# DanielBrosch/SDPSymmetryReduction.jl

Measured on AMD Instinct MI355X. Metric: N x N SDP reductions/sec (admissible_subspace+blockDiagonalize) at N=4096, higher is better.
Workload: dtype int8 square (int32 acc) + f64 eigen

## Files before the change

### include/sdpsr.h

```cpp
#ifndef SDPSR_H
#define SDPSR_H

#include <stddef.h>
#include <stdint.h>

#ifdef __cplusplus
extern "C" {
#endif

#define SDPSR_VERSION_MAJOR 0
#define SDPSR_VERSION_MINOR 5

typedef struct sdpsr_ctx sdpsr_ctx;
typedef struct sdpsr_problem sdpsr_problem;

typedef enum sdpsr_status {
    SDPSR_OK = 0,
    SDPSR_INVALID_DECOMPOSITION_FIELD = 1,
    SDPSR_NUMERICAL_INCONSISTENCY = 2,
    SDPSR_DIMENSION_MISMATCH = 3,
    SDPSR_LABEL_OVERFLOW = 4,
    SDPSR_BAD_ARGUMENT = 5,
    SDPSR_HIP_ERROR = 6,
    SDPSR_SOLVER_ERROR = 7,
    SDPSR_OUT_OF_MEMORY = 8,
    SDPSR_NOT_CONVERGED = 9,
    SDPSR_BAD_STATE = 10
} sdpsr_status;

typedef enum sdpsr_mem { SDPSR_MEM_HOST = 0, SDPSR_MEM_DEVICE = 1 } sdpsr_mem;

typedef enum sdpsr_square_mode {
    SDPSR_SQUARE_AUTO = 0,
    SDPSR_SQUARE_I8 = 1,
    SDPSR_SQUARE_F32 = 2,
    SDPSR_SQUARE_F64 = 3
} sdpsr_square_mode;

typedef enum sdpsr_round_mode {
    SDPSR_ROUND_NEAREST = 0,
    SDPSR_ROUND_TRUNC = 1
} sdpsr_round_mode;

enum {
    SDPSR_FLAG_SEPARATE_REFINEMENTS = 1u << 0,
    SDPSR_FLAG_FRESH_IRREDUCIBLE_ELEMENT = 1u << 1,
    SDPSR_FLAG_ALWAYS_REORTHOGONALIZE = 1u << 2,
    SDPSR_FLAG_REFINE_NO_FUSE = 1u << 3,
    SDPSR_FLAG_UNPACK_EVERY_STEP = 1u << 4,
    SDPSR_FLAG_SPMM_ONE_BY_ONE = 1u << 5,
    SDPSR_FLAG_SINGLE_COUPLING_ELEMENT = 1u << 6,
    SDPSR_FLAG_SMALL_EIGEN_ON_DEVICE = 1u << 7,
    SDPSR_FLAG_NO_GRAPH = 1u << 8,
    SDPSR_FLAG_NO_VERIFY_SHORTCUT = 1u << 9,
    SDPSR_FLAG_FULL_BASIS_IMAGE = 1u << 10,
    SDPSR_FLAG_ALWAYS_PROJECT = 1u << 11,
    SDPSR_FLAG_SYTRD_PANELS = 1u << 12,
    SDPSR_FLAG_COUPLING_ON_HOST = 1u << 13,
    SDPSR_FLAG_SYTRD_ONE_LAUNCH = 1u << 14,
    SDPSR_FLAG_WAIT_FOR_EVERY_VERDICT = 1u << 15,
    SDPSR_FLAG_WIDE_LOOP_LABELS = 1u << 16,
    SDPSR_FLAG_MODULE_SCRATCH_FILLS = 1u << 17,
    SDPSR_FLAG_SQUARE_EVERY_VERDICT = 1u << 18,
    SDPSR_FLAG_CHECKS_IN_LOOP = 1u << 19,
    SDPSR_FLAG_LABELS_BEFORE_BLOCKDIAG = 1u << 20
};

typedef struct sdpsr_opts {
    uint32_t struct_size;
    int32_t square_mode;
    int32_t channels;
    int32_t max_iters;
    int32_t confirm_rounds;
    int32_t eig_driver;
    uint32_t flags;
    int32_t round_mode;
    int32_t basis_image_kernel;
    int32_t refine_path;
    int32_t label_bits;
    int32_t insert_wgs_per_cu;
    int32_t square_kernel;
    int32_t reserved[3];
} sdpsr_opts;

enum {
    SDPSR_T_TOTAL = 0,
    SDPSR_T_PROJECT = 1,
    SDPSR_T_SQUARE = 2,
    SDPSR_T_REFINE = 3,
    SDPSR_T_EIGEN = 4,
    SDPSR_T_ISO = 5,
    SDPSR_T_IRRED = 6,
    SDPSR_T_IMAGE = 7,
    SDPSR_T_COUNT = 8
};

int sdpsr_create(int device_id, uint64_t seed, const sdpsr_opts* opts, sdpsr_ctx** out);
void sdpsr_destroy(sdpsr_ctx* ctx);
const char* sdpsr_last_error(const sdpsr_ctx* ctx);
const char* sdpsr_status_string(int status);
int sdpsr_version(void);
int sdpsr_set_stream(sdpsr_ctx* ctx, void* hip_stream);
int sdpsr_synchronize(sdpsr_ctx* ctx);
int sdpsr_wait_stream(sdpsr_ctx* ctx, void* hip_stream);
int sdpsr_hint_symmetric_basis(sdpsr_ctx* ctx, int yes);
int sdpsr_set_seed(sdpsr_ctx* ctx, uint64_t seed);
int sdpsr_dimension_trajectory(sdpsr_ctx* ctx, int64_t* dims, int32_t capacity, int32_t* count);

int sdpsr_set_label_width(sdpsr_ctx* ctx, int bits);
int sdpsr_label_width(sdpsr_ctx* ctx);
int sdpsr_labels_convert(sdpsr_ctx* ctx, int64_t len, const void* in, int in_bits, void* out, int out_bits, int mem);

int sdpsr_partition_from_f64(sdpsr_ctx* ctx, int64_t len, const double* M,
                             uint32_t* labels, int64_t* nparts, int mem);
int sdpsr_partition_from_u32(sdpsr_ctx* ctx, int64_t len, const uint32_t* in,
                             uint32_t* labels, int64_t* nparts, int mem);
int sdpsr_partition_from_u64(sdpsr_ctx* ctx, int64_t len, const uint64_t* in,
                             uint32_t* labels, int64_t* nparts, int mem);
// ... 164 lines not shown
```

### include/sdpsr_prof.h

```cpp
#ifndef SDPSR_PROF_H
#define SDPSR_PROF_H

#include "sdpsr.h"

#ifdef __cplusplus
extern "C" {
#endif

int sdpsr_profile_kernel(sdpsr_ctx* ctx, int kind, int64_t n, int64_t aux, int reps,
                         double* ms_per_launch);
int sdpsr_profile_clock(sdpsr_ctx* ctx, int kind, int64_t n, int64_t aux, int reps, double* out);
int sdpsr_profile_host_waits(sdpsr_ctx* ctx, uint64_t* out);
int sdpsr_profile_loop_counts(sdpsr_ctx* ctx, int32_t restart, uint64_t* out);
int sdpsr_profile_band_chase(sdpsr_ctx* ctx, int64_t n, int b, const double* A_host, double* d_host, double* e_host, double* out);
int sdpsr_profile_band_reduce(sdpsr_ctx* ctx, int64_t n, int b, double* A_host, double* out);
int sdpsr_profile_sytrd_graphs(sdpsr_ctx* ctx, double* out);
int sdpsr_profile_gather_packed(sdpsr_ctx* ctx, int64_t n, int T, int64_t d, uint64_t key, const uint32_t* Lp_host, const uint32_t* Lfull_host,
                                int8_t* X_plain, int8_t* X_writing, int8_t* X_full, uint32_t* L_inout, int64_t guard);
int sdpsr_profile_verify(sdpsr_ctx* ctx, int64_t n, int T, int64_t d, int mode, const uint32_t* Lp_host, const uint32_t* first_idx_host,
                         const int32_t* C_host, const double* U_host, double coef, uint64_t key, double atol, uint32_t* out);
int sdpsr_profile_basis_constant(sdpsr_ctx* ctx, int64_t n, int r, int64_t d, const uint32_t* Lp_host, const uint32_t* first_idx_host,
                                 const double* U_host, double atol, uint32_t* out);
int sdpsr_profile_verify_pair(sdpsr_ctx* ctx, int64_t n, int64_t d, const uint32_t* Lp_host, const uint32_t* first_idx_host,
                              const double* a_host, const double* b_host, uint32_t* out);
int sdpsr_profile_initial_guess(sdpsr_ctx* ctx, int32_t restart, uint64_t* out);
int sdpsr_profile_narrow_labels(sdpsr_ctx* ctx, int32_t restart, uint64_t* out);
int sdpsr_profile_gather_packed_w(sdpsr_ctx* ctx, int64_t n, int T, int64_t d, uint64_t key, int width, const uint32_t* Lp_host, int8_t* X_plain,
                                  int8_t* X_writing, uint32_t* L_inout, int64_t guard);
int sdpsr_profile_verify_w(sdpsr_ctx* ctx, int64_t n, int T, int64_t d, int r, int width, const uint32_t* Lp_host, const uint32_t* first_idx_host,
                           const int32_t* C_host, const double* U_host, const double* coef_host, uint64_t key, double atol, uint32_t* out);
int sdpsr_profile_verify_pair_w(sdpsr_ctx* ctx, int64_t n, int64_t d, int width, const uint32_t* Lp_host, const uint32_t* first_idx_host,
                                const double* a_host, const double* b_host, uint32_t* out);
int sdpsr_profile_proj_coef_lower(sdpsr_ctx* ctx, int64_t n, int64_t r, uint64_t key, int width, const uint32_t* Lp_host, const double* U_host,
                                  double* partial_out, double* coef_out);
int sdpsr_profile_refine_source(sdpsr_ctx* ctx, int kind, int what, int64_t n, int64_t ld, int T, int r, int packed, int lab_packed, uint64_t key,
                                double atol, const double* a_host, const double* b_host, const double* U_host, const double* coef_host,
                                const void* C_host, uint32_t* L_inout, uint32_t* Lnew_inout, int64_t guard, int64_t prev_classes, int sym,
                                uint64_t* sig_out, int64_t* nparts, uint32_t* first_out, int32_t* report);
int sdpsr_profile_square_checks(sdpsr_ctx* ctx, int32_t restart, uint64_t* out);
int sdpsr_profile_deferred_checks(sdpsr_ctx* ctx, int32_t restart, uint64_t* out);
int sdpsr_profile_recorded_labels(sdpsr_ctx* ctx, int32_t restart, uint64_t* out);
int sdpsr_profile_square_check(sdpsr_ctx* ctx, int64_t n, int64_t d, int G, int T, const uint64_t* keys, int width, int write_full,
                               const uint32_t* Lp_host, const uint32_t* first_idx_host, uint8_t* ws_inout, uint64_t* layout,
                               uint32_t* verdicts_out, uint32_t* L_inout, int64_t guard);


int sdpsr_profile_gram(sdpsr_ctx* ctx, int mode, int64_t k, int64_t ma, int64_t nb, int64_t lda, int64_t ldb, int64_t mp, int64_t np,
                       const double* A_host, const double* B_host, double* C_inout, double* pinned_inout, int64_t guard, int32_t* report);
int sdpsr_profile_tall_times_small(sdpsr_ctx* ctx, int64_t n, int64_t ldi, int64_t kk, int64_t lds, int64_t ncols, double alpha, double beta,
                                   int64_t ldo, const double* In_host, const double* S_host, double* out_inout, int64_t guard);
int sdpsr_profile_label_product(sdpsr_ctx* ctx, int64_t n, int64_t d, int G, int64_t w, int64_t ldw, int64_t ldy, const uint64_t* keys,
                                const uint32_t* L_host, const double* W_host, double* Y_inout, int64_t guard, int32_t* report);
int sdpsr_profile_label_product_pair(sdpsr_ctx* ctx, int64_t n, int64_t d, int64_t w, int64_t ldw, int64_t ldy, const uint64_t* keys,
                                     const uint32_t* L_host, const double* W_host, double* Y0_inout, double* Y1_inout, int64_t guard,
                                     int32_t* report);
int sdpsr_profile_class_sums2(sdpsr_ctx* ctx, int64_t n, int64_t d, uint32_t first, int plain, const uint32_t* L_host, const double* X_host,
                              double* Y_inout, int64_t guard, int32_t* report);
int sdpsr_profile_class_sums(sdpsr_ctx* ctx, int64_t n, int64_t d, int64_t ldo, const uint32_t* L_host, const double* x_host,
                             double* out_inout, int64_t guard, int32_t* report);
int sdpsr_profile_symmetrize(sdpsr_ctx* ctx, int64_t m, int64_t ld, double* B_inout, int64_t guard);
int sdpsr_profile_extract_symmetric(sdpsr_ctx* ctx, int64_t m, int64_t mp, int64_t lds, const double* src_host, double* dst_inout, int64_t guard);
int sdpsr_profile_normalize_columns(sdpsr_ctx* ctx, int64_t n, int64_t ldx, int64_t hstride, int64_t nruns, const double* X_host,
                                    double* H_inout, double* norm_inout, int64_t guard);
int sdpsr_profile_random_vector(sdpsr_ctx* ctx, int64_t n, uint64_t key, double* x_inout, int64_t guard);


int sdpsr_profile_poison_scratch(sdpsr_ctx* ctx);
int sdpsr_profile_stacked_in_place(sdpsr_ctx* ctx, int64_t n, int64_t ldi, int64_t kk, int64_t lds, int64_t ncols, int64_t w, int64_t mcols,
                                   double* M_inout, const double* S_host, int64_t guard, int32_t* report);
int sdpsr_profile_lift(sdpsr_ctx* ctx, int64_t n, int64_t ldi, int64_t kk, int64_t lds, int64_t S1, double atol, const double* In_host,
                       const double* S_host, double* Qcm_inout, double* Qrm_inout, int64_t guard);
int sdpsr_profile_seed_vector(sdpsr_ctx* ctx, int64_t n, uint64_t key, double* x_inout, double* h_inout, double* norm_inout, int64_t guard);
int sdpsr_profile_qrm_current(sdpsr_ctx* ctx, int32_t* current);


int sdpsr_profile_cx_gather_herm(sdpsr_ctx* ctx, int64_t n, const uint32_t* L_host, uint64_t key, double* Hr_inout, double* Hi_inout, int64_t guard);
int sdpsr_profile_cx_heev(sdpsr_ctx* ctx, int route, int64_t n, const double* Hr_host, const double* Hi_host, double atol, double* w_inout,
                          double* Vr_inout, double* Vi_inout, int64_t guard, int32_t* info_out);
int sdpsr_profile_cx_block_norms(sdpsr_ctx* ctx, int route, int64_t n, const double* Hr_host, const double* Hi_host, const double* Vr_host,
                                 const double* Vi_host, const int32_t* space_of, int32_t neig, double* norms_inout, int64_t guard);
int sdpsr_profile_cx_irreducible(sdpsr_ctx* ctx, int route, int64_t n, int64_t vcols, const double* Hr_host, const double* Hi_host,
                                 const double* Vr_host, const double* Vi_host, const int32_t* desc, int32_t ncols, double atol,
                                 double* Qhat_inout, int64_t guard);


int sdpsr_profile_dense_block_norms(sdpsr_ctx* ctx, int route, int64_t n, int64_t ld, const double* A_host, const double* Q_host,
                                    const int32_t* space_of, int32_t neig, double* norms_inout, double* M_inout, double* T_inout, int64_t guard);
int sdpsr_profile_dense_cluster_norms(sdpsr_ctx* ctx, int64_t n, int64_t ld, const double* A_host, const double* Q_host,
                                      const double* evals_host, double atol, const int32_t* einfo, void* pack_inout, double* T_inout, int64_t guard);
int sdpsr_profile_dense_classes(sdpsr_ctx* ctx, int32_t neig, double* norms_inout, const int32_t* dims_host, double atol, uint64_t* stat_out,
                                double* edges_out, double* thr_out, uint64_t* bits_inout, int32_t* kpart_out, int64_t guard);
int sdpsr_profile_dense_irreducible(sdpsr_ctx* ctx, int route, int64_t n, int64_t ldq, int64_t vcols, const double* Q_host, const double* Bf_host,
                                    int64_t nf, const int32_t* desc, int32_t npairs, double* Qhat_inout, int64_t ncols, int64_t guard,
                                    int32_t* report);
int sdpsr_profile_copy_cols(sdpsr_ctx* ctx, int64_t n, int64_t count, const int32_t* src_cols, const int32_t* dst_cols, const double* src_host,
                            int64_t ld_src, int64_t scols, double* dst_inout, int64_t ld_dst, int64_t dcols, int64_t guard);
int sdpsr_profile_clamptol(sdpsr_ctx* ctx, int64_t len, double* a_inout, double atol, int64_t guard);


int sdpsr_profile_sytrd(sdpsr_ctx* ctx, int64_t n, int64_t ld, double* A_inout, double* d_inout, double* e_inout, double* tau_inout,
                        int64_t guard);
int sdpsr_profile_backtransform(sdpsr_ctx* ctx, int64_t n, int64_t ld, const double* A_host, const double* tau_host, double* Z_inout,
                                int64_t guard);
int sdpsr_profile_stedc(sdpsr_ctx* ctx, int64_t n, int64_t ld, const double* d_host, const double* e_host, double* w_inout, double* Z_inout,
                        int64_t guard);

#ifdef __cplusplus
}
#endif
#endif
// ... 1 lines not shown
```

### sdpsymmetryreduction.jl_amd/_lib.py

```python
from __future__ import annotations

import ctypes as C
import os
import re

import numpy as np

_HERE = os.path.dirname(os.path.abspath(__file__))
LIB_PATH = os.path.join(_HERE, "libsdpsr_hip.so")
PROF_LIB_PATH = os.path.join(_HERE, "libsdpsr_prof.so")
HEADER_PATH = os.path.join(os.path.dirname(_HERE), "include", "sdpsr.h")
PROF_HEADER_PATH = os.path.join(os.path.dirname(_HERE), "include", "sdpsr_prof.h")

MEM_HOST, MEM_DEVICE = 0, 1
SQUARE_AUTO, SQUARE_I8, SQUARE_F32, SQUARE_F64 = 0, 1, 2, 3
T_TOTAL, T_PROJECT, T_SQUARE, T_REFINE, T_EIGEN, T_ISO, T_IRRED, T_IMAGE, T_COUNT = range(9)
ROUND_NEAREST, ROUND_TRUNC = 0, 1
SETUP_NO_CONSTRAINTS, SETUP_CHOLESKY_QR2, SETUP_MGS = 0, 1, 2
FLAG_SEPARATE_REFINEMENTS = 1 << 0
FLAG_FRESH_IRREDUCIBLE_ELEMENT = 1 << 1
FLAG_ALWAYS_REORTHOGONALIZE = 1 << 2
FLAG_REFINE_NO_FUSE = 1 << 3
FLAG_UNPACK_EVERY_STEP = 1 << 4
FLAG_SPMM_ONE_BY_ONE = 1 << 5
FLAG_SINGLE_COUPLING_ELEMENT = 1 << 6
FLAG_SMALL_EIGEN_ON_DEVICE = 1 << 7
FLAG_NO_GRAPH = 1 << 8
FLAG_NO_VERIFY_SHORTCUT = 1 << 9
FLAG_FULL_BASIS_IMAGE = 1 << 10
FLAG_ALWAYS_PROJECT = 1 << 11
FLAG_SYTRD_PANELS = 1 << 12
FLAG_COUPLING_ON_HOST = 1 << 13
FLAG_SYTRD_ONE_LAUNCH = 1 << 14
FLAG_WAIT_FOR_EVERY_VERDICT = 1 << 15
FLAG_WIDE_LOOP_LABELS = 1 << 16
FLAG_MODULE_SCRATCH_FILLS = 1 << 17
FLAG_SQUARE_EVERY_VERDICT = 1 << 18
FLAG_CHECKS_IN_LOOP = 1 << 19
FLAG_LABELS_BEFORE_BLOCKDIAG = 1 << 20
BASIS_IMAGE_KERNELS = {"auto": 0, "two_stage": 1, "outer": 2, "chunk": 3}
BI_ROUTE_COMMUTATIVE, BI_ROUTE_BLOCKS, BI_ROUTE_TWO_STAGE, BI_ROUTE_OUTER, BI_ROUTE_CHUNK = 1, 2, 3, 4, 5
BI_ROUTE_REPAIRED, BI_ROUTE_SHORTCUT_REFUSED = 0x100, 0x200
TRI_UPPER, TRI_FULL = 0, 1
REFINE_PATHS = {"auto": 0, "hash": 1, "sort": 2, "bucket": 3, "no_mid": 4, "mid_no_first": 6}

LABEL_DTYPES = {8: np.dtype(np.uint8), 16: np.dtype(np.uint16), 32: np.dtype(np.uint32)}


def label_dtype(bits):
    try:
        return LABEL_DTYPES[int(bits)]
    except KeyError:
        raise ValueError(f"label width must be 8, 16 or 32, not {bits!r}") from None


STATUS = {
    0: "OK", 1: "INVALID_DECOMPOSITION_FIELD", 2: "NUMERICAL_INCONSISTENCY", 3: "DIMENSION_MISMATCH",
    4: "LABEL_OVERFLOW", 5: "BAD_ARGUMENT", 6: "HIP_ERROR", 7: "SOLVER_ERROR", 8: "OUT_OF_MEMORY",
    9: "NOT_CONVERGED", 10: "BAD_STATE",
}


class Opts(C.Structure):
    _fields_ = [
        ("struct_size", C.c_uint32),
        ("square_mode", C.c_int32),
        ("channels", C.c_int32),
        ("max_iters", C.c_int32),
        ("confirm_rounds", C.c_int32),
        ("eig_driver", C.c_int32),
        ("flags", C.c_uint32),
        ("round_mode", C.c_int32),
        ("basis_image_kernel", C.c_int32),
        ("refine_path", C.c_int32),
        ("label_bits", C.c_int32),
        ("insert_wgs_per_cu", C.c_int32),
        ("square_kernel", C.c_int32),
        ("reserved", C.c_int32 * 3),
    ]


def declared_symbols(header_path=HEADER_PATH):
    txt = open(header_path).read()
    txt = re.sub(r"/\*.*?\*/", "", txt, flags=re.S)
    return sorted(set(re.findall(r"\b(sdpsr_[a-z0-9_]+)\s*\(", txt)))


_lib = None


def load_library():
    global _lib
# ... 106 lines not shown


_prof = None


def load_prof_library():
    global _prof
    if _prof is not None:
        return _prof
    load_library()
    if not os.path.exists(PROF_LIB_PATH):
        raise RuntimeError(f"{PROF_LIB_PATH} is missing: build it with `make -C sdpsymmetryreduction.jl_amd/csrc`")
    lib = C.CDLL(PROF_LIB_PATH)
    vp, i64 = C.c_void_p, C.c_int64
    for name in ("sdpsr_profile_kernel", "sdpsr_profile_clock"):
        fn = getattr(lib, name)
        fn.restype = C.c_int
        fn.argtypes = [vp, C.c_int, i64, i64, C.c_int, C.POINTER(C.c_double)]
    lib.sdpsr_profile_band_chase.restype = C.c_int
    lib.sdpsr_profile_band_chase.argtypes = [vp, i64, C.c_int, vp, vp, vp, C.POINTER(C.c_double)]
    lib.sdpsr_profile_band_reduce.restype = C.c_int
    lib.sdpsr_profile_band_reduce.argtypes = [vp, i64, C.c_int, vp, C.POINTER(C.c_double)]
    lib.sdpsr_profile_host_waits.restype = C.c_int
    lib.sdpsr_profile_host_waits.argtypes = [vp, C.POINTER(C.c_uint64)]
    lib.sdpsr_profile_loop_counts.restype = C.c_int
    lib.sdpsr_profile_loop_counts.argtypes = [vp, C.c_int32, C.POINTER(C.c_uint64)]
    lib.sdpsr_profile_sytrd_graphs.restype = C.c_int
    lib.sdpsr_profile_sytrd_graphs.argtypes = [vp, C.POINTER(C.c_double)]
    lib.sdpsr_profile_gather_packed.restype = C.c_int
    lib.sdpsr_profile_gather_packed.argtypes = [vp, i64, C.c_int, i64, C.c_uint64, vp, vp, vp, vp, vp, vp, i64]
    lib.sdpsr_profile_verify.restype = C.c_int
    lib.sdpsr_profile_verify.argtypes = [vp, i64, C.c_int, i64, C.c_int, vp, vp, vp, vp, C.c_double, C.c_uint64, C.c_double,
                                         C.POINTER(C.c_uint32)]
    lib.sdpsr_profile_basis_constant.restype = C.c_int
    lib.sdpsr_profile_basis_constant.argtypes = [vp, i64, C.c_int, i64, vp, vp, vp, C.c_double, C.POINTER(C.c_uint32)]
    lib.sdpsr_profile_verify_pair.restype = C.c_int
    lib.sdpsr_profile_verify_pair.argtypes = [vp, i64, i64, vp, vp, vp, vp, C.POINTER(C.c_uint32)]
    lib.sdpsr_profile_initial_guess.restype = C.c_int
    lib.sdpsr_profile_initial_guess.argtypes = [vp, C.c_int32, C.POINTER(C.c_uint64)]
    lib.sdpsr_profile_narrow_labels.restype = C.c_int
    lib.sdpsr_profile_narrow_labels.argtypes = [vp, C.c_int32, C.POINTER(C.c_uint64)]
    lib.sdpsr_profile_gather_packed_w.restype = C.c_int
    lib.sdpsr_profile_gather_packed_w.argtypes = [vp, i64, C.c_int, i64, C.c_uint64, C.c_int, vp, vp, vp, vp, i64]
    lib.sdpsr_profile_verify_w.restype = C.c_int
    lib.sdpsr_profile_verify_w.argtypes = [vp, i64, C.c_int, i64, C.c_int, C.c_int, vp, vp, vp, vp, vp, C.c_uint64, C.c_double, C.POINTER(C.c_uint32)]
    lib.sdpsr_profile_verify_pair_w.restype = C.c_int
    lib.sdpsr_profile_verify_pair_w.argtypes = [vp, i64, i64, C.c_int, vp, vp, vp, vp, C.POINTER(C.c_uint32)]
    lib.sdpsr_profile_square_checks.restype = C.c_int
    lib.sdpsr_profile_square_checks.argtypes = [vp, C.c_int32, C.POINTER(C.c_uint64)]
    lib.sdpsr_profile_deferred_checks.restype = C.c_int
    lib.sdpsr_profile_deferred_checks.argtypes = [vp, C.c_int32, C.POINTER(C.c_uint64)]
    lib.sdpsr_profile_recorded_labels.restype = C.c_int
    lib.sdpsr_profile_recorded_labels.argtypes = [vp, C.c_int32, C.POINTER(C.c_uint64)]
    lib.sdpsr_profile_square_check.restype = C.c_int
    lib.sdpsr_profile_square_check.argtypes = [vp, i64, i64, C.c_int, C.c_int, vp, C.c_int, C.c_int, vp, vp, vp, vp, vp, vp, i64]
    lib.sdpsr_profile_proj_coef_lower.restype = C.c_int
    lib.sdpsr_profile_proj_coef_lower.argtypes = [vp, i64, i64, C.c_uint64, C.c_int, vp, vp, vp, vp]
    lib.sdpsr_profile_refine_source.restype = C.c_int
    lib.sdpsr_profile_refine_source.argtypes = [vp, C.c_int, C.c_int, i64, i64, C.c_int, C.c_int, C.c_int, C.c_int, C.c_uint64, C.c_double,
                                                vp, vp, vp, vp, vp, vp, vp, i64, i64, C.c_int, vp, C.POINTER(i64), vp, C.POINTER(C.c_int32)]
    f64, rep = C.c_double, C.POINTER(C.c_int32)
    lib.sdpsr_profile_gram.restype = C.c_int
    lib.sdpsr_profile_gram.argtypes = [vp, C.c_int, i64, i64, i64, i64, i64, i64, i64, vp, vp, vp, vp, i64, rep]
    lib.sdpsr_profile_tall_times_small.restype = C.c_int
    lib.sdpsr_profile_tall_times_small.argtypes = [vp, i64, i64, i64, i64, i64, f64, f64, i64, vp, vp, vp, i64]
    lib.sdpsr_profile_label_product.restype = C.c_int
    lib.sdpsr_profile_label_product.argtypes = [vp, i64, i64, C.c_int, i64, i64, i64, vp, vp, vp, vp, i64, rep]
    lib.sdpsr_profile_label_product_pair.restype = C.c_int
    lib.sdpsr_profile_label_product_pair.argtypes = [vp, i64, i64, i64, i64, i64, vp, vp, vp, vp, vp, i64, rep]
    lib.sdpsr_profile_class_sums2.restype = C.c_int
    lib.sdpsr_profile_class_sums2.argtypes = [vp, i64, i64, C.c_uint32, C.c_int, vp, vp, vp, i64, rep]
    lib.sdpsr_profile_class_sums.restype = C.c_int
    lib.sdpsr_profile_class_sums.argtypes = [vp, i64, i64, i64, vp, vp, vp, i64, rep]
    lib.sdpsr_profile_symmetrize.restype = C.c_int
    lib.sdpsr_profile_symmetrize.argtypes = [vp, i64, i64, vp, i64]
    lib.sdpsr_profile_extract_symmetric.restype = C.c_int
    lib.sdpsr_profile_extract_symmetric.argtypes = [vp, i64, i64, i64, vp, vp, i64]
    lib.sdpsr_profile_normalize_columns.restype = C.c_int
    lib.sdpsr_profile_normalize_columns.argtypes = [vp, i64, i64, i64, i64, vp, vp, vp, i64]
    lib.sdpsr_profile_random_vector.restype = C.c_int
    lib.sdpsr_profile_random_vector.argtypes = [vp, i64, C.c_uint64, vp, i64]
    lib.sdpsr_profile_poison_scratch.restype = C.c_int
    lib.sdpsr_profile_poison_scratch.argtypes = [vp]
    lib.sdpsr_profile_stacked_in_place.restype = C.c_int
    lib.sdpsr_profile_stacked_in_place.argtypes = [vp, i64, i64, i64, i64, i64, i64, i64, vp, vp, i64, rep]
    lib.sdpsr_profile_lift.restype = C.c_int
    lib.sdpsr_profile_lift.argtypes = [vp, i64, i64, i64, i64, i64, f64, vp, vp, vp, vp, i64]
    lib.sdpsr_profile_seed_vector.restype = C.c_int
    lib.sdpsr_profile_seed_vector.argtypes = [vp, i64, C.c_uint64, vp, vp, vp, i64]
    lib.sdpsr_profile_qrm_current.restype = C.c_int
    lib.sdpsr_profile_qrm_current.argtypes = [vp, rep]
    lib.sdpsr_profile_cx_gather_herm.restype = C.c_int
    lib.sdpsr_profile_cx_gather_herm.argtypes = [vp, i64, vp, C.c_uint64, vp, vp, i64]
    lib.sdpsr_profile_cx_heev.restype = C.c_int
    lib.sdpsr_profile_cx_heev.argtypes = [vp, C.c_int, i64, vp, vp, f64, vp, vp, vp, i64, rep]
    lib.sdpsr_profile_cx_block_norms.restype = C.c_int
    lib.sdpsr_profile_cx_block_norms.argtypes = [vp, C.c_int, i64, vp, vp, vp, vp, vp, C.c_int32, vp, i64]
    lib.sdpsr_profile_cx_irreducible.restype = C.c_int
    lib.sdpsr_profile_cx_irreducible.argtypes = [vp, C.c_int, i64, i64, vp, vp, vp, vp, vp, C.c_int32, f64, vp, i64]
    lib.sdpsr_profile_dense_block_norms.restype = C.c_int
    lib.sdpsr_profile_dense_block_norms.argtypes = [vp, C.c_int, i64, i64, vp, vp, vp, C.c_int32, vp, vp, vp, i64]
    lib.sdpsr_profile_dense_cluster_norms.restype = C.c_int
    lib.sdpsr_profile_dense_cluster_norms.argtypes = [vp, i64, i64, vp, vp, vp, f64, vp, vp, vp, i64]
    lib.sdpsr_profile_dense_classes.restype = C.c_int
    lib.sdpsr_profile_dense_classes.argtypes = [vp, C.c_int32, vp, vp, f64, vp, vp, vp, vp, vp, i64]
    lib.sdpsr_profile_dense_irreducible.restype = C.c_int
# ... 14 lines not shown
```

### sdpsymmetryreduction.jl_amd/csrc/blockdiag.cpp

```cpp
#include <algorithm>
#include <cmath>
#include <cstdio>
#include <cstdlib>
#include <cstring>

#include "host_internal.h"

using namespace sdpsr;

namespace sdpsr {
static int keep_labels(sdpsr_ctx* c, int64_t n, const uint32_t* P, int mem, bool trusted_symmetric, bool in_place, bool labels_are_u32,
                       uint32_t*& L) {
    hipStream_t s = c->stream;
    const int64_t len = n * n;
    int st = SDPSR_OK;
    const bool narrow = !labels_are_u32 && c->label_width != 32;
    in_place = in_place && mem == SDPSR_MEM_DEVICE && !narrow;
    L = in_place ? const_cast<uint32_t*>(P) : (uint32_t*)ctx_buf(c, "bd_labels", len * 4);
    if (!L) return SDPSR_OUT_OF_MEMORY;
    c->bd_labels_ext = in_place ? P : nullptr;
    c->bd_sym_labels = nullptr;
    c->bd_sym_epoch = 0;
    c->bd_trusted_symmetric = (trusted_symmetric && mem == SDPSR_MEM_DEVICE && P == L) ? L : nullptr;
    if (narrow) {
        st = labels_fetch(c, L, P, (size_t)len, mem);
        if (st) return st;
    } else if (mem == SDPSR_MEM_DEVICE) {
        if (P != L) {
            const bool fresh = c->bufs.find("bd_symflag") == c->bufs.end();
            uint32_t* sf = (uint32_t*)ctx_buf(c, "bd_symflag", 64);
            if (!sf) return SDPSR_OUT_OF_MEMORY;
            if (fresh) HIP_TRY(c, hipMemsetAsync(sf, 0, 64, s));
            if (++c->epoch_counter == 0) ++c->epoch_counter;
            launch_copy_check_symmetric(s, n, P, L, sf, c->epoch_counter);
            c->bd_sym_epoch = c->epoch_counter;
            c->bd_sym_labels = L;
        }
    } else {
        HIP_TRY(c, hipMemcpyAsync(L, P, len * 4, hipMemcpyHostToDevice, s));
        c->h2d_bytes += (size_t)len * 4;
    }
    return SDPSR_OK;
}

static int check_block_sizes(sdpsr_ctx* c, const std::vector<int32_t>& sizes, int64_t d) {
    int64_t final_dim = 0;
    for (int32_t sz : sizes) final_dim += (int64_t)sz * (sz + 1) / 2;
    if (final_dim == d) return SDPSR_OK;
    std::string szs;
    for (int32_t sz : sizes) szs += std::to_string(sz) + " ";
    return ctx_fail(c, SDPSR_DIMENSION_MISMATCH,
                    "final_dim=" + std::to_string(final_dim) + " block_sizes=[" + szs + "] expected dim(P)=" +
                        std::to_string(d) + " (rounding error: try another epsilon or try again; or the algebra is not block-diagonalizable over the reals)");
}

int block_diagonalize_impl(sdpsr_ctx* c, int64_t n, const uint32_t* P, int64_t d, double epsilon, int32_t* nblocks, int64_t* sum_sq,
                           int64_t* sum_s, double* phase_ms, int mem, bool trusted_symmetric, bool final_sync, bool in_place, bool labels_are_u32) {
    CHECK_CTX(c);
    if (!P || n < 1 || d < 0 || !(epsilon > 0)) return ctx_fail(c, SDPSR_BAD_ARGUMENT, "bad arguments");
    const int64_t len = n * n;
    int st = check_len(c, len);
    if (st) return st;
    hipStream_t s = c->stream;
    c->bd_valid = false;
    c->bd_q_valid = false;
    c->bd_qrm_current = false;
    PhaseTimer tm(c, phase_ms != nullptr);
    TotalEvents ev_total(phase_ms != nullptr, s);
    uint32_t* L = nullptr;
    st = keep_labels(c, n, P, mem, trusted_symmetric, in_place, labels_are_u32, L);
    if (st) return st;
    dbg_mark(c, "block_diagonalize: entered, labels copied");
    const double atol = epsilon;
    EigInfo info;
    std::vector<int32_t> sizes;
    int64_t S1 = 0, S = 0;
    st = DRIVER_FALLBACK;
    if (compression_eligible(c, n, d)) st = compressed_diagonalize(c, n, L, d, atol, info, sizes, S1, S, tm);
    if (st == DRIVER_FALLBACK && c->opts.eig_driver == 6)
        return ctx_fail(c, SDPSR_SOLVER_ERROR, "requested driver not applicable to this partition (" + c->err + ")");
    if (st != SDPSR_OK && st != DRIVER_FALLBACK) return st;
    if (st == DRIVER_FALLBACK) {
        flush_deferred_tail(c);
        st = dense_diagonalize(c, n, L, nullptr, atol, info, sizes, S1, S, tm, d);
        if (st) return st;
    }

    dbg_mark(c, "block_diagonalize: diagonalize done");
    c->bd_n = n;
    c->bd_d = d;
    c->bd_sizes = sizes;
    c->bd_sum_s = S1;
    c->bd_sum_sq = S;
    c->bd_q_valid = true;
    if (nblocks) *nblocks = (int32_t)sizes.size();
    if (sum_sq) *sum_sq = S;
    if (sum_s) *sum_s = S1;
    if (phase_ms) {
        const float ms = ev_total.stop(s);
        tm.collect();
        for (int i = 0; i < SDPSR_T_COUNT; ++i) phase_ms[i] = tm.acc[i];
        phase_ms[SDPSR_T_TOTAL] = ms;
    } else if (final_sync) {
        HIP_TRY(c, ctx_sync_stream(c, s));
    }
    st = check_block_sizes(c, sizes, d);
    if (st) return st;
    c->bd_valid = true;
    return SDPSR_OK;
}

struct BasisImage {
    enum Shortcut { FALL_THROUGH, DONE, DONE_SYNCED };
    enum Route { TWO_STAGE, OUTER, CHUNK };
    sdpsr_ctx* c;
    hipStream_t s;
    int64_t n, d, S1, S, len;
    uint32_t first;
    const uint32_t* L;
    const double* Qrm;
    double* out;
    double atol;
    const std::vector<int32_t>& sizes;
// ... 298 lines not shown
```

### sdpsymmetryreduction.jl_amd/csrc/compress.cpp

```cpp
#include <algorithm>
#include <cmath>
#include <cstdio>
#include <cstring>
#include <functional>

#include "host_internal.h"
#include "module_select.h"

using namespace sdpsr;

namespace {

struct Rider { double *dBs, *gps; bool have_t; };

struct Module {
    sdpsr_ctx* c;
    int64_t n, ld, d;
    const uint32_t* L;
    int wmax;
    int64_t wcap, ycap, wtot;
    double *W = nullptr, *T = nullptr, *zy = nullptr, *dout = nullptr, *Cc = nullptr, *dSm = nullptr, *Q1 = nullptr;
    int w = 1;
    std::vector<double> hG;
    int64_t saved_ld = 0;
// ... 137 lines not shown
            return ctx_fail(c, SDPSR_INVALID_DECOMPOSITION_FIELD,
                            "partition is not symmetric: decomposition over Float64 requested but the generic element has a complex spectrum");
    }
    sel = select_directions(hG.data(), ap, w, mc, tol, take_ref);
    return SDPSR_OK;
}

int Module::apply_stacked(int mc, const Selection& sel) {
    int e2 = h2d_sync(c, dSm, sel.coef.data(), (size_t)(w + mc) * sel.rank * 8);
    if (e2) return e2;
    double* V = W + (size_t)w * ld;
    const bool in_place = !parent_form() && launch_tall_times_small_rows(c->stream, n, ld, W, w + mc, dSm, w + mc, sel.rank, 1.0, 0.0, V, ld);
    if (!in_place) {
        live = mc;
        e2 = restore_fills();
        if (e2) return e2;
        launch_tall_times_small(c->stream, n, ld, W, w + mc, dSm, w + mc, sel.rank, 1.0, 0.0, Q1, ld);
        HIP_TRY(c, hipMemcpyAsync(V, Q1, (size_t)ld * sel.rank * 8, hipMemcpyDeviceToDevice, c->stream));
    }
    live = sel.rank;
    return SDPSR_OK;
}

int Module::absorb(int m, const Rider* rider, int& got) {
    got = 0;
    Selection s1, s2;
    int st = ortho_step(m, 1e-10, true, rider, s1);
    if (st) return st;
    if (dbg_on() && s1.rank > 0) fprintf(stderr, "[sdpsr] absorb(%d): rank %d, pivots %.3e .. %.3e (ratio %.1e)\n", m, s1.rank, s1.piv_max, s1.piv_min, s1.piv_max / s1.piv_min);
    first_product_intact = (s1.rank == 0);
    if (s1.rank == 0) return SDPSR_OK;
    if (w + s1.rank >= wmax) return driver_fallback(c, "module dimension exceeds " + std::to_string(wmax));
    st = apply_stacked(m, s1);
    if (st) return st;
    const double worst = std::max(s1.piv_max, s1.ref) / s1.piv_min;
    got = s1.rank;
    if (!(worst <= 1e3) || (c->opts.flags & SDPSR_FLAG_ALWAYS_REORTHOGONALIZE)) {
        st = ortho_step(s1.rank, 1e-6, false, nullptr, s2);
        got = s2.rank;
        if (st || got == 0) return st;
        st = apply_stacked(s1.rank, s2);
        if (st) return st;
    }
    w += got;
    live = 0;
    return SDPSR_OK;
}

int Module::class_sum_round() {
    if (!(class_sums_supports(n, d, ld) && basis_image_two_stage_fits(n, d, 1) && d <= ycap && d + 1 < wmax)) {
        flush_deferred_tail(c);
        return SDPSR_OK;
    }
    launch_class_sums(c->stream, n, d, L, W, W + (size_t)w * ld, ld);
    window = 0;
    int got;
    live = (int)d;
    return absorb((int)d, nullptr, got);
}

int Module::growth_round(int& got) {
    const bool fused = fused_product(w);
    int G = (fused && w <= 16) ? 4 : 2;
    while (G > 2 && (int64_t)G * w > ycap) --G;
    if ((int64_t)G * w > ycap || w >= d) G = 1;
    const int m = G * w;
    double* Y = W + (size_t)w * ld;
    live = 0;
    window = 1;
    deferred_window_close(c);
    if (lean && !(fused && small_on_host())) {
        const int e0 = restore_fills();
        if (e0) return e0;
    }
    if (!lean) HIP_TRY(c, hipMemsetAsync(Y, 0, (size_t)ld * round_up(m, 128) * 8, c->stream));
    bool batched = false;
    if (fused && G > 1 && G != 3 && G * w <= 64 && !(c->opts.flags & SDPSR_FLAG_SPMM_ONE_BY_ONE)) {
        double* part = (double*)ctx_buf(c, "cm_part", label_spmm_pair_partial_doubles(n) * 8);
        if (!part) return SDPSR_OUT_OF_MEMORY;
        uint64_t keys[4];
        const uint64_t save = c->stream_counter;
        for (int gidx = 0; gidx < G; ++gidx) keys[gidx] = next_key(c);
        batched = launch_label_spmm_multi(c->stream, n, L, keys, G, d, W, ld, w, part, Y, ld);
        if (!batched) c->stream_counter = save;
    }
    spec_b2 = false;
    Rider rider{};
    bool armed = false;
    if (G == 1 && small_on_host()) {
        char* pinb = (char*)ctx_pinned(c, spec_b2_offset() + (size_t)w * w * 8);
        rider.dBs = (double*)ctx_buf(c, "cm_bsmall", (size_t)64 * 64 * 8);
        rider.gps = (double*)ctx_buf(c, "gram_partials", gram_small_partial_doubles(n, 128, 128) * 8);
        armed = pinb && rider.dBs && rider.gps;
    }
    if (armed && fused && !(c->opts.flags & SDPSR_FLAG_SPMM_ONE_BY_ONE)) {
        double* part = (double*)ctx_buf(c, "cm_part", label_spmm_pair_partial_doubles(n) * 8);
        if (!part) return SDPSR_OUT_OF_MEMORY;
        uint64_t keys[2];
        const uint64_t save = c->stream_counter;
        keys[0] = next_key(c);
        keys[1] = next_key(c);
        rider.have_t = launch_label_spmm_pair(c->stream, n, L, keys, d, W, ld, w, part, Y, ld, T, ld);
        if (!rider.have_t) c->stream_counter = save;
    }
    for (int gidx = 0; gidx < G && !batched && !rider.have_t; ++gidx) {
        live = gidx * w;
        int e2 = apply_generic(w, Y + (size_t)gidx * w * ld);
// ... 198 lines not shown
```

### sdpsymmetryreduction.jl_amd/csrc/ctx.cpp

```cpp
#include <algorithm>
#include <cmath>
#include <complex>
#include <cstdio>
#include <cstdlib>
#include <cstring>
#include <chrono>
#include <functional>
#include <numeric>

#include "host_internal.h"

using namespace sdpsr;
int ctx_fail(sdpsr_ctx* c, int status, const std::string& msg) {
    if (c) c->err = std::string(sdpsr_status_string(status)) + ": " + msg;
    return status;
}

void* ctx_buf(sdpsr_ctx* c, const char* name, size_t bytes) {
    if (bytes == 0) bytes = 16;
    auto it = c->bufs.find(std::string_view(name));
    if (it != c->bufs.end() && it->second.bytes >= bytes) return it->second.p;
    DevBuf& b = it != c->bufs.end() ? it->second : c->bufs[std::string(name)];
    const std::string_view nm(name);
    if (nm == "adm_lpacked" || nm == "adm_lpacked8" || nm == "ref_first" || nm == "adm_lfull_rec") c->initial_record = InitialRecord{};
    if (nm == "adm_symflag") c->symflag_zero = false;
    if (nm == "bd_qhat" || nm == "bd_qrm") c->bd_qrm_current = false;
    if (b.p) {
        flush_deferred_tail(c);
        ctx_sync_stream(c, c->stream);
        hipFree(b.p);
        b.p = nullptr;
        b.bytes = 0;
    }
    size_t want = bytes + (bytes >> 3);
    want = (want + 255) & ~size_t(255);
    if (hipMalloc(&b.p, want) != hipSuccess) {
        b.p = nullptr;
        if (hipMalloc(&b.p, bytes) != hipSuccess) {
            b.p = nullptr;
            ctx_fail(c, SDPSR_OUT_OF_MEMORY, std::string("hipMalloc ") + name + " " + std::to_string(bytes));
            return nullptr;
        }
        want = bytes;
    }
    b.bytes = want;
    return b.p;
}


namespace sdpsr {
uint64_t steady_ns() {
    return (uint64_t)std::chrono::duration_cast<std::chrono::nanoseconds>(std::chrono::steady_clock::now().time_since_epoch()).count();
}
void* ctx_pinned(sdpsr_ctx* c, size_t bytes) {
    if (c->pinned_bytes >= bytes) return c->pinned;
    ctx_sync_stream(c, c->stream);
    if (c->pinned) hipHostFree(c->pinned);
    c->pinned = nullptr;
    c->pinned_bytes = 0;
    size_t want = std::max<size_t>(bytes + bytes / 4, 1 << 16);
    if (hipHostMalloc(&c->pinned, want, hipHostMallocCoherent) != hipSuccess) {
        c->pinned = nullptr;
        return nullptr;
    }
    c->pinned_bytes = want;
    return c->pinned;
}

bool ctx_ensure_side(sdpsr_ctx* c) {
    if (!c->side_stream && hipStreamCreateWithFlags(&c->side_stream, hipStreamNonBlocking) != hipSuccess) {
        c->side_stream = nullptr;
        (void)hipGetLastError();
        return false;
    }
    hipEvent_t* evs[] = {&c->ev_fork, &c->ev_join, &c->ev_bt_fork, &c->ev_bt_join};
    for (hipEvent_t* e : evs)
        if (!*e && hipEventCreateWithFlags(e, hipEventDisableTiming) != hipSuccess) {
// ... 257 lines not shown
```

### sdpsymmetryreduction.jl_amd/csrc/host_internal.h

```cpp
#pragma once
#include <algorithm>
#include <cstring>
#include <functional>
#include <string>
#include <vector>

#include "agree_plan.h"
#include "csr_canon.h"
#include "iso_classes.h"
#include "sdpsr_internal.h"

struct sdpsr_comm {
    int device = 0;
    int32_t world = 1, rank = 0;
    void* nccl = nullptr;
};

namespace sdpsr {

bool dbg_on();
void dbg_mark(sdpsr_ctx* c, const char* what);

struct DeviceGuard {
    int prev = -1;
// ... 189 lines not shown
constexpr PinnedWords PINNED_VERIFY{128, 1};
constexpr PinnedWords PINNED_SPECULATIVE{144, 1};
constexpr PinnedWords PINNED_BASIS_CONSTANT{192, 1};
constexpr PinnedWords PINNED_SAMPLE{224, 4};
constexpr size_t PINNED_FIXED_BYTES = 1024;
constexpr PinnedWords PINNED_BASIS_IMAGE_VERDICTS{64, 1};
constexpr PinnedWords PINNED_SMALL_FLAG{0, 1};
constexpr PinnedWords PINNED_SMALL_LABEL_CHECK{2, 2};
constexpr PinnedWords PINNED_SMALL_ROWSPACE_NNZ{4, 2};
constexpr PinnedWords PINNED_SMALL_DEFERRED_VERIFY{8, 1};
constexpr PinnedWords PINNED_SMALL_DEFERRED_SPECULATIVE{24, 1};
constexpr PinnedWords PINNED_SMALL_DEFERRED_INITIAL{16, 1};
constexpr PinnedWords PINNED_SMALL_DEFERRED_NARROW{20, 1};
constexpr PinnedWords PINNED_SMALL_GRAM_STAMP{32, 1};
constexpr PinnedWords PINNED_SMALL_CANON{44, 18};
constexpr PinnedWords PINNED_SMALL_NARROW{40, 1};
constexpr bool pinned_words_disjoint(std::initializer_list<PinnedWords> w, size_t bytes) {
    for (const PinnedWords* a = w.begin(); a != w.end(); ++a) {
        if (a->count == 0 || (a->first + a->count) * 4 > bytes) return false;
        for (const PinnedWords* b = w.begin(); b != a; ++b)
            if (a->first < b->first + b->count && b->first < a->first + a->count) return false;
    }
    return true;
}
static_assert(pinned_words_disjoint({PINNED_REFINE, PINNED_SYMMETRY, PINNED_BASIS_IMAGE_VERDICTS, PINNED_VERIFY, PINNED_SPECULATIVE, PINNED_BASIS_CONSTANT, PINNED_SAMPLE}, PINNED_FIXED_BYTES) &&
              PINNED_FIXED_BYTES % sizeof(double) == 0, "two reports share a word of c->pinned, or one reaches into the symmetry probe's doubles");
static_assert(pinned_words_disjoint({PINNED_SMALL_FLAG, PINNED_SMALL_LABEL_CHECK, PINNED_SMALL_ROWSPACE_NNZ, PINNED_SMALL_DEFERRED_VERIFY, PINNED_SMALL_DEFERRED_SPECULATIVE, PINNED_SMALL_DEFERRED_INITIAL, PINNED_SMALL_DEFERRED_NARROW, PINNED_SMALL_GRAM_STAMP, PINNED_SMALL_NARROW, PINNED_SMALL_CANON}, 256) &&
              (PINNED_SMALL_CANON.first * 4) % 8 == 0 && PINNED_SMALL_CANON.count * 4 == sizeof(CanonVerdict), "two reports share a word of c->pinned_small");
inline uint32_t* pinned_report(sdpsr_ctx* c, PinnedWords w) {
    uint32_t* p = (uint32_t*)ctx_pinned(c, PINNED_FIXED_BYTES);
    return p ? p + w.first : nullptr;
}
inline uint32_t initial_guess_violated(const sdpsr_ctx* c) {
    const volatile uint32_t* ps = c->pinned_small;
    return ps[PINNED_SMALL_DEFERRED_INITIAL.first] | ps[PINNED_SMALL_DEFERRED_NARROW.first];
}

int refine_signatures(sdpsr_ctx* c, int64_t len, const SigSource& src_in, uint32_t* labels, int64_t* nparts, int64_t sym_n = 0,
                      uint32_t* symflag_dev = nullptr, int* sym_out = nullptr, bool early = false);
int refine_signatures(sdpsr_ctx* c, int64_t len, const uint64_t* sig, uint32_t* labels, int64_t* nparts, int64_t sym_n = 0,
                      uint32_t* symflag_dev = nullptr, int* sym_out = nullptr, bool early = false);

int admissible_subspace_impl(sdpsr_ctx* c, int64_t n, const double* CL, const double* X0L, const double* U, int64_t r, double atol,
                             uint32_t* P_out, int64_t* dim_out, int32_t* iters_out, double* phase_ms, int mem, int mem_out,
                             bool final_sync, int* labels_sym_out);
int setup_mgs(sdpsr_ctx* c, int64_t len, int64_t m, double* R, double* U, double* partial, int nblk, double* coef,
              std::vector<std::vector<double>>& coeffs, std::vector<int64_t>& piv, int64_t* r_out);
std::vector<double> min_norm_coefficients(int64_t r, const std::vector<int64_t>& piv, const std::vector<std::vector<double>>& coeffs,
                                          const double* b);
int setup_tail(sdpsr_ctx* c, int64_t n, int64_t r, const double* U, const std::vector<double>& y, double atol, double* v1, double* v2,
               double* dCL, double* dX0, double* partial, int nblk, double* coef);
int block_diagonalize_impl(sdpsr_ctx* c, int64_t n, const uint32_t* P, int64_t d, double epsilon, int32_t* nblocks, int64_t* sum_sq,
                           int64_t* sum_s, double* phase_ms, int mem, bool trusted_symmetric, bool final_sync, bool in_place = false,
                           bool labels_are_u32 = true);

struct EigInfo {
    std::vector<double> vals;
    std::vector<int> ptrs;
    std::vector<int> kpart;
    bool t_valid = false;
};

struct ElemGen {
    std::function<int(double* dst)> make;
    std::function<int(double* dst)> prefetch;
    std::function<int()> join;
    std::function<int()> fork;
};
int make_element(sdpsr_ctx* c, const ElemGen* gen, int64_t n, int64_t ld, const uint32_t* L, double* dst);
int isomorphism_classes(sdpsr_ctx* c, const std::vector<double>& norms, int neig, double atol, std::vector<int>& kpart);
struct CouplingTrace {
    double edges[17];
    double thr;
};
int isomorphism_classes_device(sdpsr_ctx* c, unsigned long long* dnorms, int neig, const std::vector<int32_t>& dims, double atol,
                               std::vector<int>& kpart, CouplingTrace* trace = nullptr);
void couple_block_norms(hipStream_t s, int64_t n, int64_t ld, double* Ap, const double* Q, double* Tp, const int32_t* dspace, int neig,
                        unsigned long long* dnorms);
bool irreducible_pairs_fit_lds(int64_t max_m2);
int irreducible_pairs(sdpsr_ctx* c, int64_t n, int64_t ld, const double* Q, const double* Bf, const std::vector<int32_t>& pairs,
                      int64_t max_m2, double* Qhat, int route = -1, int* ran = nullptr);
int irreducible_pairs_one_by_one(sdpsr_ctx* c, int64_t n, int64_t ld, const double* Q, const double* Bf, const std::vector<int32_t>& pairs,
                                 double* Qhat);
int eigen_decomposition_device(sdpsr_ctx* c, int64_t n, const uint32_t* L, double atol, EigInfo& info, PhaseTimer& tm,
                               const ElemGen* gen = nullptr, int64_t expect_dim = -1);
constexpr int DRIVER_FALLBACK = -1000;
int driver_fallback(sdpsr_ctx* c, const std::string& why);
int dense_diagonalize(sdpsr_ctx* c, int64_t n, const uint32_t* L, const ElemGen* gen, double atol, EigInfo& info,
                      std::vector<int32_t>& sizes, int64_t& S1, int64_t& S, PhaseTimer& tm, int64_t expect_dim = -1);
int gemm_tn_splitk(sdpsr_ctx* c, int64_t m, int64_t n, int64_t k, const double* A, int64_t lda, const double* B, int64_t ldb,
                   double* C, int64_t ldc, const char* partials = "splitk_partials");
bool gram_tn_is_skinny(int64_t ma, int64_t nb);
int gram_tn(sdpsr_ctx* c, int64_t ma, int64_t nb, int64_t k, const double* A, int64_t lda, const double* B, int64_t ldb, double* C,
            int64_t mp, int64_t np, double* host_C = nullptr, bool* host_filled = nullptr);
int compressed_diagonalize(sdpsr_ctx* c, int64_t n, const uint32_t* L, int64_t d, double atol, EigInfo& info,
                           std::vector<int32_t>& sizes, int64_t& S1, int64_t& S, PhaseTimer& tm);
bool compression_eligible(const sdpsr_ctx* c, int64_t n, int64_t d);

int host_syev(int n, const double* A, int lda, double* w, double* Z, int ldz);
void host_count_edges17(const double* x, size_t n, const double* ed, int64_t* hist);
void host_gemm_tn(int m, int n, int k, const double* A, int lda, const double* B, int ldb, double* C, int ldc);
int murota_small_host(sdpsr_ctx* c, int w, const double* B1, const std::function<int(double*)>& next_element, double atol,
                      int64_t expect_dim, std::vector<int32_t>& sizes, int64_t& S1, int64_t& S, std::vector<double>& Qs);

void launch_symmetrize(hipStream_t s, int64_t m, int64_t ld, double* B);
void launch_extract_symmetric(hipStream_t s, int64_t m, int64_t mp, const double* src, int64_t lds_, double* dst);
void launch_splitk_reduce(hipStream_t s, int64_t len, int Z, int64_t stride, const double* P, double* C);
// ... 109 lines not shown
```

### sdpsymmetryreduction.jl_amd/csrc/kernels_blockdiag.hip

```cpp
#include <cstdlib>
#include <type_traits>
#include "host_internal.h"
#include "kernel_util.h"

namespace sdpsr {

typedef double v4d __attribute__((ext_vector_type(4)));

__global__ void block_norms_kernel(int64_t n, int64_t ld, const double* __restrict__ M,
                                   const int32_t* __restrict__ space_of, int neig,
                                   unsigned long long* __restrict__ norms) {
    const int64_t len = n * n;
    const int64_t stride = (int64_t)gridDim.x * blockDim.x;
    for (int64_t e0 = (int64_t)blockIdx.x * blockDim.x; e0 < len; e0 += stride) {
        const int64_t e = e0 + threadIdx.x;
        bool valid = e < len;
        int64_t j = valid ? e / n : 0, i = valid ? e - j * n : 0;
        int bi = space_of[i], bj = space_of[j];
        unsigned long long v = valid ? (unsigned long long)__double_as_longlong(fabs(M[i + j * ld])) : 0ull;
        int key = bi * neig + bj;
        int prev_key = __shfl_up(key, 1, 64);
        bool head = ((threadIdx.x & 63) == 0) || prev_key != key;
#pragma unroll
        for (int o = 1; o < 64; o <<= 1) {
// ... 688 lines not shown
                    for (int g2 = 1; g2 < groups; ++g2) tot += __shfl(t, jl + g2 * sub, 64);
                    t = tot;
                }
                if (act && g == 0) {
                    if (lower && diag == (uint32_t)i) t = fma(0.5, Qrm[(int64_t)r * S1 + (int64_t)j * VEC + v], t);
                    T[((int64_t)(i - 1) * nn + r) * S1 + (int64_t)j * VEC + v] = t;
                }
            }
        }
    }
}

__global__ void __launch_bounds__(256)
basis_image_blocks_kernel(int n, int S1, int64_t S, const double* __restrict__ Qrm, const double* __restrict__ T,
                          const int32_t* __restrict__ colA, const int32_t* __restrict__ colB, double atol,
                          double* __restrict__ out) {
    __shared__ double red[256];
    const int i = blockIdx.x;
    const int64_t o = (int64_t)blockIdx.y * 4 + (threadIdx.x & 3);
    const int g = threadIdx.x >> 2;
    const double* Ti = T + (int64_t)i * n * S1;
    double a0 = 0, a1 = 0;
    if (o < S) {
        const int ca = colA[o], cb = colB[o];
        int r = g;
        for (; r + 64 < n; r += 128) {
            const double qa0 = Qrm[(int64_t)r * S1 + ca], qb0 = Qrm[(int64_t)r * S1 + cb];
            const double ta0 = Ti[(int64_t)r * S1 + ca], tb0 = Ti[(int64_t)r * S1 + cb];
            const double qa1 = Qrm[(int64_t)(r + 64) * S1 + ca], qb1 = Qrm[(int64_t)(r + 64) * S1 + cb];
            const double ta1 = Ti[(int64_t)(r + 64) * S1 + ca], tb1 = Ti[(int64_t)(r + 64) * S1 + cb];
            a0 = fma(qa0, tb0, a0);
            a0 = fma(qb0, ta0, a0);
            a1 = fma(qa1, tb1, a1);
            a1 = fma(qb1, ta1, a1);
        }
        for (; r < n; r += 64) {
            a0 = fma(Qrm[(int64_t)r * S1 + ca], Ti[(int64_t)r * S1 + cb], a0);
            a0 = fma(Qrm[(int64_t)r * S1 + cb], Ti[(int64_t)r * S1 + ca], a0);
        }
    }
    red[threadIdx.x] = a0 + a1;
    __syncthreads();
    if (threadIdx.x < 4 && o < S) {
        double v = 0;
        for (int gg = 0; gg < 64; ++gg) v += red[gg * 4 + threadIdx.x];
        out[(int64_t)i * S + o] = (fabs(v) < atol) ? 0.0 : v;
    }
}

bool basis_image_two_stage_fits(int64_t n, int64_t d, int64_t S1) {
    return n <= 65535 && (2 * (d + 2) * 4 + n * 2) <= 60 * 1024 && d * n * S1 * 8 <= ((int64_t)4 << 30);
}

__global__ void __launch_bounds__(256)
class_sums_small_d_kernel(int n, int d, uint32_t first, int tstride, const uint32_t* __restrict__ L, const double* __restrict__ x,
                          double* __restrict__ out, int64_t ldo) {
    extern __shared__ __attribute__((aligned(16))) double cs_smem[];
    double* sx = cs_smem;
    const int lane = threadIdx.x & 63, wave = threadIdx.x >> 6;
    double* acc = cs_smem + n + (size_t)wave * 64 * tstride;
    double* mine = acc + (size_t)lane * tstride;
    for (int c = threadIdx.x; c < n; c += 256) sx[c] = x[c];
    __syncthreads();
    const int rows_per_round = gridDim.x * 4;
    const int bpr = (n + 511) / 512;
    const int my_rows = (n - blockIdx.x * 4 + rows_per_round - 1) / rows_per_round;
    const int total = my_rows * bpr;
    auto fetch = [&](int bq, uint32_t (&lab)[8]) {
        const int rr = bq / bpr, bb = bq - rr * bpr;
        const int r = blockIdx.x * 4 + rr * rows_per_round + wave;
        const uint32_t* col = L + (int64_t)((bq < total && r < n) ? r : 0) * n;
#pragma unroll
        for (int u = 0; u < 8; ++u) {
            const int c = bb * 512 + u * 64 + lane;
            lab[u] = col[c < n ? c : n - 1];
        }
    };
    auto process = [&](int bq, const uint32_t (&lab)[8]) {
        if (bq >= total) return;
        const int rr = bq / bpr, bb = bq - rr * bpr;
        if (bb == 0)
            for (int i = 0; i <= d; ++i) mine[i] = 0.0;
        double vv[8];
#pragma unroll
        for (int u = 0; u < 8; ++u) {
            const int c = bb * 512 + u * 64 + lane;
            vv[u] = c < n ? sx[c] : 0.0;
        }
#pragma unroll
        for (int u = 0; u < 8; ++u) atomicAdd(&mine[window_label(lab[u], first, (uint32_t)d)], vv[u]);
        if (bb == bpr - 1) {
            const int r = blockIdx.x * 4 + rr * rows_per_round + wave;
            __syncthreads();
            if (r < n)
                for (int i = 1 + lane; i <= d; i += 64) {
                    double t = 0;
                    for (int l2 = 0; l2 < 64; ++l2) t += acc[(size_t)l2 * tstride + i];
                    out[(int64_t)(i - 1) * ldo + r] = t;
                }
            __syncthreads();
        }
    };
    uint32_t qa[8], qb[8], qc[8], qd[8];
    fetch(0, qa);
    fetch(1, qb);
    fetch(2, qc);
#pragma unroll 1
    for (int bq = 0; bq < total; bq += 4) {
        fetch(bq + 3, qd);
        process(bq, qa);
        fetch(bq + 4, qa);
        process(bq + 1, qb);
        fetch(bq + 5, qb);
        process(bq + 2, qc);
        fetch(bq + 6, qc);
        process(bq + 3, qd);
    }
}

__device__ __forceinline__ double bi_weight(uint64_t key, int k) {
    return 0.5 + (double)(sdpsr_fmix64(key + 0x9E3779B97F4A7C15ULL * (uint64_t)(k + 1)) >> 11) * (1.0 / 9007199254740992.0);
}

__global__ void bi_signed_sums_kernel(int n, int S1, const double* __restrict__ Qrm, uint64_t key, double2* __restrict__ X, uint32_t* flag) {
    const int r = blockIdx.x * blockDim.x + threadIdx.x;
    if (blockIdx.x == 0)
        for (int k = threadIdx.x; k <= S1; k += blockDim.x) flag[k] = 0u;
    if (r >= n) return;
    double a = 0, b = 0;
    for (int k = 0; k < S1; ++k) {
        const double q = Qrm[(int64_t)r * S1 + k];
        a += q;
        b = fma(bi_weight(key, k), q, b);
    }
    X[r] = make_double2(a, b);
}

__global__ void bi_pair_vector_kernel(int n, int S1, const double* __restrict__ Qrm, int k1, int k2, double2* __restrict__ X) {
    const int r = blockIdx.x * blockDim.x + threadIdx.x;
    if (r < n) X[r] = make_double2(Qrm[(int64_t)r * S1 + k1], Qrm[(int64_t)r * S1 + k2]);
}

__global__ void __launch_bounds__(256)
bi_contract_pair_kernel(int n, int S1, const double* __restrict__ Qrm, const double2* __restrict__ Y, int k1, int k2, double atol,
                        double* __restrict__ out) {
    __shared__ double red[2][256];
    const int i = blockIdx.x;
    const double2* Yi = Y + (int64_t)i * n;
    double a0 = 0, a1 = 0;
    for (int r = threadIdx.x; r < n; r += 256) {
        const double2 y = Yi[r];
        a0 = fma(Qrm[(int64_t)r * S1 + k1], y.x, a0);
        a1 = fma(Qrm[(int64_t)r * S1 + k2], y.y, a1);
    }
    red[0][threadIdx.x] = a0;
    red[1][threadIdx.x] = a1;
    __syncthreads();
    if (threadIdx.x < 2) {
        double v = 0;
        for (int g = 0; g < 256; ++g) v += red[threadIdx.x][g];
        const int k = threadIdx.x == 0 ? k1 : k2;
        out[(int64_t)i * S1 + k] = (fabs(v) < atol) ? 0.0 : v;
    }
}

template <int W, bool WIN>
__global__ void __launch_bounds__(64 * W)
class_sums2_kernel(int n, int d, uint32_t first, int tstride, const uint32_t* __restrict__ L, const double2* __restrict__ X,
                   double2* __restrict__ out) {
    extern __shared__ __attribute__((aligned(16))) double2 cs2_smem[];
    const int lane = threadIdx.x & 63, wave = threadIdx.x >> 6;
    double2* acc = cs2_smem + (size_t)wave * 64 * tstride;
    double2* mine = acc + (size_t)lane * tstride;
    const int rows_per_round = gridDim.x * W;
    const int bpr = (n + 511) / 512;
    const int my_rows = (n - (int)blockIdx.x * W + rows_per_round - 1) / rows_per_round;
    const int total = my_rows * bpr;
    auto fetch = [&](int bq, uint32_t (&lab)[8], double2 (&xv)[8]) {
        const int rr = bq / bpr, bb = bq - rr * bpr;
        const int r = blockIdx.x * W + rr * rows_per_round + wave;
        const uint32_t* col = L + (int64_t)((bq < total && r < n) ? r : 0) * n;
#pragma unroll
        for (int u = 0; u < 8; ++u) {
            const int c = bb * 512 + u * 64 + lane;
            const int cc = c < n ? c : n - 1;
            lab[u] = col[cc];
            xv[u] = X[cc];
        }
    };
    auto process = [&](int bq, const uint32_t (&lab)[8], const double2 (&xv)[8]) {
        if (bq >= total) return;
        const int rr = bq / bpr, bb = bq - rr * bpr;
        if (bb == 0)
            for (int i = 0; i <= d; ++i) mine[i] = make_double2(0.0, 0.0);
#pragma unroll
        for (int u = 0; u < 8; ++u) {
            const int c = bb * 512 + u * 64 + lane;
            if (c < n) {
                const uint32_t l = WIN ? window_label(lab[u], first, (uint32_t)d) : lab[u];
                double2 t = mine[l];
                t.x += xv[u].x;
                t.y += xv[u].y;
                mine[l] = t;
            }
        }
        if (bb == bpr - 1) {
            const int r = blockIdx.x * W + rr * rows_per_round + wave;
            __syncthreads();
            if (r < n)
                for (int i = 1 + lane; i <= d; i += 64) {
                    double tx = 0, ty = 0;
                    for (int l2 = 0; l2 < 64; ++l2) {
                        const double2 v = acc[(size_t)l2 * tstride + i];
                        tx += v.x;
                        ty += v.y;
                    }
                    out[(int64_t)(i - 1) * n + r] = make_double2(tx, ty);
                }
            __syncthreads();
        }
    };
    uint32_t la[8], lb[8], lc[8];
    double2 xa[8], xb[8], xc[8];
    fetch(0, la, xa);
    fetch(1, lb, xb);
#pragma unroll 1
    for (int bq = 0; bq < total; bq += 3) {
        fetch(bq + 2, lc, xc);
        process(bq, la, xa);
        fetch(bq + 3, la, xa);
        process(bq + 1, lb, xb);
        fetch(bq + 4, lb, xb);
        process(bq + 2, lc, xc);
    }
}

__global__ void __launch_bounds__(256)
bi_contract_check_kernel(int n, int S1, const double* __restrict__ Qrm, const double2* __restrict__ Y, uint64_t key, double atol,
                         double tol, double* __restrict__ out, uint32_t* __restrict__ flag) {
    __shared__ double red[2][256];
    const int i = blockIdx.x;
    const int k = blockIdx.y * 4 + (threadIdx.x & 3);
    const int g = threadIdx.x >> 2;
    const double2* Yi = Y + (int64_t)i * n;
    double a0 = 0, a1 = 0;
    if (k < S1)
        for (int r0 = g; r0 < n; r0 += 64 * 8) {
            double q[8];
            double2 y[8];
#pragma unroll
            for (int x = 0; x < 8; ++x) {
                const int r = r0 + 64 * x;
                const int rc = r < n ? r : g;
                q[x] = r < n ? Qrm[(int64_t)rc * S1 + k] : 0.0;
                y[x] = Yi[rc];
            }
#pragma unroll
            for (int x = 0; x < 8; ++x) {
                a0 = fma(q[x], y[x].x, a0);
                a1 = fma(q[x], y[x].y, a1);
            }
        }
    red[0][threadIdx.x] = a0;
    red[1][threadIdx.x] = a1;
    __syncthreads();
    if (threadIdx.x < 4 && k < S1) {
        double v0 = 0, v1 = 0;
        for (int gg = 0; gg < 64; ++gg) {
            v0 += red[0][gg * 4 + threadIdx.x];
            v1 += red[1][gg * 4 + threadIdx.x];
        }
        if (!(fabs(v0 - v1 / bi_weight(key, k)) <= tol)) {
            if (atomicExch(&flag[1 + k], 1u) == 0u) atomicAdd(&flag[0], 1u);
        }
        out[(int64_t)i * S1 + k] = (fabs(v0) < atol) ? 0.0 : v0;
    }
}

static void launch_class_sums2(hipStream_t s, int W, int g, size_t lds, int64_t n, int64_t d, uint32_t first, bool plain, int tstride, const uint32_t* L,
                               const double2* X, double2* Y) {
    if (plain && first == 1u) {
        if (W == 4) class_sums2_kernel<4, false><<<g, 256, lds, s>>>((int)n, (int)d, first, tstride, L, X, Y);
        else if (W == 2) class_sums2_kernel<2, false><<<g, 128, lds, s>>>((int)n, (int)d, first, tstride, L, X, Y);
        else class_sums2_kernel<1, false><<<g, 64, lds, s>>>((int)n, (int)d, first, tstride, L, X, Y);
    } else {
        if (W == 4) class_sums2_kernel<4, true><<<g, 256, lds, s>>>((int)n, (int)d, first, tstride, L, X, Y);
        else if (W == 2) class_sums2_kernel<2, true><<<g, 128, lds, s>>>((int)n, (int)d, first, tstride, L, X, Y);
// ... 173 lines not shown
        }
        Bs[a2][b2] = v;
    }
    __syncthreads();
    if (only < 0 && threadIdx.x < 12) {
        const int a2 = threadIdx.x % 3, t = sz + threadIdx.x / 3;
        if (a2 < sz && t < BIB_T) {
            double v = 0;
            for (int b2 = 0; b2 < sz; ++b2) v += Bs[a2][b2] * bib_weight(key, k, b2, t, sz);
            if (!(fabs(v - ys[a2][t]) <= tol)) s_bad = 1;
        }
    }
    __syncthreads();
    if (threadIdx.x == 0 && s_bad && atomicExch(&flag[1 + k], 1u) == 0u) atomicAdd(&flag[0], 1u);
    if (threadIdx.x < 9) {
        const int a2 = threadIdx.x / 3, b2 = threadIdx.x % 3;
        if (a2 < sz && b2 < sz) {
            const double v = 0.5 * (Bs[a2][b2] + Bs[b2][a2]);
            out[(int64_t)i * S + blk_off[k] + a2 + b2 * sz] = (fabs(v) < atol) ? 0.0 : v;
        }
    }
}
size_t basis_image_blocks_workspace_doubles(int64_t n, int64_t d) { return (size_t)4 * n * (d + 1) + 9 * 65536; }
bool launch_basis_image_blocks(hipStream_t s, int64_t n, int64_t d, uint32_t first, int64_t S1, int64_t S, int nblocks, const int32_t* blk_col, const int32_t* blk_size,
                               const int64_t* blk_off, const uint32_t* L, const double* Qrm, uint64_t key, int only, double atol, double tol, double* ws,
                               double* out, uint32_t* flag, bool plain) {
    const int tstride = (int)((d + 1) | 1);
    const size_t per_wave = (size_t)64 * tstride * sizeof(double2);
    int W = 4;
    while (W > 1 && per_wave * W > 150 * 1024) W >>= 1;
    if (per_wave * W > 150 * 1024 || n < 1 || n > 0x7FFFFFFF / 2 || nblocks < 1 || nblocks > 65535) return false;
    double2* X0 = reinterpret_cast<double2*>(ws);
    double2* X1 = X0 + n;
    double2* Y0 = X1 + n;
    double2* Y1 = Y0 + (size_t)d * n;
    double* ginv = reinterpret_cast<double*>(Y1 + (size_t)d * n);
    if ((size_t)S1 * BIB_T * 8 > 48 * 1024) return false;
    bib_vectors_kernel<<<(unsigned)((n + 255) / 256), 256, (size_t)S1 * BIB_T * 8, s>>>((int)n, (int)S1, nblocks, blk_col, blk_size, key, only, Qrm, X0, X1, only < 0 ? flag : nullptr, ginv);
    int g = (int)((n + W - 1) / W);
    if (g > 256) g = 256;
    const size_t lds = per_wave * W;
    for (int pass = 0; pass < 2; ++pass) {
        const double2* X = pass ? X1 : X0;
        double2* Y = pass ? Y1 : Y0;
        launch_class_sums2(s, W, g, lds, n, d, first, plain, tstride, L, X, Y);
    }
    dim3 gc((unsigned)d, only >= 0 ? 1u : (unsigned)nblocks);
    bib_contract_kernel<<<gc, 256, 0, s>>>((int)n, (int)S1, S, blk_col, blk_size, blk_off, Qrm, Y0, Y1, ginv, key, only, atol, tol, out, flag);
    return true;
}

bool blockdiag_set_device_attributes() {
    bool ok = true;
    ok &= hipSuccess == hipFuncSetAttribute(reinterpret_cast<const void*>(&class_sums2_kernel<4, false>), hipFuncAttributeMaxDynamicSharedMemorySize, 150 * 1024);
    ok &= hipSuccess == hipFuncSetAttribute(reinterpret_cast<const void*>(&class_sums2_kernel<4, true>), hipFuncAttributeMaxDynamicSharedMemorySize, 150 * 1024);
    ok &= hipSuccess == hipFuncSetAttribute(reinterpret_cast<const void*>(&class_sums2_kernel<2, false>), hipFuncAttributeMaxDynamicSharedMemorySize, 150 * 1024);
    ok &= hipSuccess == hipFuncSetAttribute(reinterpret_cast<const void*>(&class_sums2_kernel<2, true>), hipFuncAttributeMaxDynamicSharedMemorySize, 150 * 1024);
    ok &= hipSuccess == hipFuncSetAttribute(reinterpret_cast<const void*>(&class_sums2_kernel<1, false>), hipFuncAttributeMaxDynamicSharedMemorySize, 150 * 1024);
    ok &= hipSuccess == hipFuncSetAttribute(reinterpret_cast<const void*>(&class_sums2_kernel<1, true>), hipFuncAttributeMaxDynamicSharedMemorySize, 150 * 1024);
    ok &= hipSuccess == hipFuncSetAttribute(reinterpret_cast<const void*>(&class_sums_small_d_kernel),
                        hipFuncAttributeMaxDynamicSharedMemorySize, 150 * 1024);
    ok &= hipSuccess == hipFuncSetAttribute(reinterpret_cast<const void*>(&small_qtaq_block_norms_kernel),
                        hipFuncAttributeMaxDynamicSharedMemorySize, 104 * 1024);
    ok &= hipSuccess == hipFuncSetAttribute(reinterpret_cast<const void*>(&small_cluster_qtaq_block_norms_kernel),
                        hipFuncAttributeMaxDynamicSharedMemorySize, 104 * 1024);
    ok &= hipSuccess == hipFuncSetAttribute(reinterpret_cast<const void*>(&basis_image_outer_mfma_kernel),
                        hipFuncAttributeMaxDynamicSharedMemorySize, 72 * 1024);
    ok &= hipSuccess == hipFuncSetAttribute(reinterpret_cast<const void*>(&basis_image_rows_kernel<1>),
                        hipFuncAttributeMaxDynamicSharedMemorySize, 64 * 1024);
    ok &= hipSuccess == hipFuncSetAttribute(reinterpret_cast<const void*>(&basis_image_rows_kernel<2>),
                        hipFuncAttributeMaxDynamicSharedMemorySize, 64 * 1024);
    return ok;
}

bool class_sums_supports(int64_t n, int64_t d, int64_t ldo) {
    const int tstride = (int)((d + 1) | 1);
    return ldo == n || ((size_t)n + (size_t)4 * 64 * tstride) * sizeof(double) <= 150 * 1024;
}
void launch_class_sums(hipStream_t s, int64_t n, int64_t d, const uint32_t* L, const double* x, double* out, int64_t ldo, uint32_t first) {
    const int tstride = (int)((d + 1) | 1);
    const size_t lds_small = ((size_t)n + (size_t)4 * 64 * tstride) * sizeof(double);
    if (lds_small <= 150 * 1024) {
        int g = (int)((n + 3) / 4);
        if (g > 256) g = 256;
        class_sums_small_d_kernel<<<g, 256, lds_small, s>>>((int)n, (int)d, first, tstride, L, x, out, ldo);
        return;
    }
    const size_t lds = (size_t)2 * (d + 2) * 4 + (size_t)n * 2 + 16;
    basis_image_rows_kernel<1><<<(unsigned)n, 64, lds, s>>>((int)n, (int)d, first, 1, L, x, out, 0);
}

void launch_basis_image_two_stage(hipStream_t s, int64_t n, int64_t d, uint32_t first, int64_t S1, int64_t S,
                                  const uint32_t* L, const double* Qrm, double* T, const int32_t* colA,
                                  const int32_t* colB, double atol, double* out) {
    const size_t lds = (size_t)2 * (d + 2) * 4 + (size_t)n * 2 + 16;
    if (S1 % 2 == 0)
        basis_image_rows_kernel<2><<<(unsigned)n, 64, lds, s>>>((int)n, (int)d, first, (int)S1, L, Qrm, T, 1);
    else
        basis_image_rows_kernel<1><<<(unsigned)n, 64, lds, s>>>((int)n, (int)d, first, (int)S1, L, Qrm, T, 1);
    dim3 g((unsigned)d, (unsigned)((S + 3) / 4));
    basis_image_blocks_kernel<<<g, 256, 0, s>>>((int)n, (int)S1, S, Qrm, T, colA, colB, atol, out);
}

__global__ void transpose_to_rowmajor_kernel(int64_t n, int64_t S1, const double* __restrict__ Qcm,
                                             double* __restrict__ Qrm) {
    const int64_t total = n * S1;
    const int64_t stride = (int64_t)gridDim.x * blockDim.x;
    for (int64_t t = (int64_t)blockIdx.x * blockDim.x + threadIdx.x; t < total; t += stride) {
        const int64_t r = t / S1, k = t - r * S1;
        Qrm[t] = Qcm[r + k * n];
    }
}
void launch_transpose_to_rowmajor(hipStream_t s, int64_t n, int64_t S1, const double* Qcm,
                                  double* Qrm) {
    transpose_to_rowmajor_kernel<<<grid_for(n * S1, 256), 256, 0, s>>>(n, S1, Qcm, Qrm);
}

__global__ void class_starts_kernel(int64_t len, const uint32_t* __restrict__ sorted_keys,
                                    int64_t* __restrict__ class_start) {
    const int64_t stride = (int64_t)gridDim.x * blockDim.x;
    for (int64_t e = (int64_t)blockIdx.x * blockDim.x + threadIdx.x; e < len; e += stride) {
        uint32_t k = sorted_keys[e];
        if (e == 0 || sorted_keys[e - 1] != k) class_start[k] = e;
    }
}

constexpr int RX_T = 256, RX_E = 8, RX_CH = RX_T * RX_E;
__device__ __forceinline__ void rx_load(int64_t len, int64_t e0, const uint32_t* __restrict__ k, const uint32_t* __restrict__ v, uint32_t first, uint32_t cnt,
                                        uint32_t (&kk)[RX_E], uint32_t (&vv)[RX_E]) {
#pragma unroll
    for (int q = 0; q < RX_E; ++q) {
        const int64_t e = e0 + q;
        kk[q] = e < len ? window_label(k[e], first, cnt) : 0xFFFFFFFFu;
        vv[q] = e < len ? (v ? v[e] : (uint32_t)e) : 0u;
    }
}
__global__ void __launch_bounds__(RX_T)
rx_hist_kernel(int64_t len, const uint32_t* __restrict__ keys, uint32_t first, uint32_t cnt, int shift, uint32_t G, uint32_t* __restrict__ hist) {
// ... 156 lines not shown
```

### sdpsymmetryreduction.jl_amd/csrc/loop.cpp

```cpp
#include <algorithm>
#include <cmath>

#include "host_internal.h"

using namespace sdpsr;

namespace {
class LoopLabels {
public:
    uint32_t* L = nullptr;
    uint32_t* Lp = nullptr;
    uint8_t* Lp8 = nullptr;
    int sym = 0;
    void init(sdpsr_ctx* ctx, int64_t order, uint32_t* symflag_dev, bool keep, bool early) { c = ctx, n = order, symflag = symflag_dev, keep_packed = keep, early_ok = early; }
    bool packed() const { return packed_valid; }
    const uint32_t* current(bool from_packed) const { return from_packed ? Lp : L; }
    void need_full() {
        if (!full_valid) launch_unpack_symmetric_labels(c->stream, n, Lp, L);
        full_valid = true;
    }
    uint32_t* full_from_gather() {
        if (full_valid || !packed_valid) return nullptr;
        full_valid = true;
        return L;
// ... 106 lines not shown
        q2.kind = SIG_CHAN_I32;
        if (!verify_no_split_supports(qj, current) || !verify_no_split_supports(q2, current)) return false;
        return ctx_buf(c, "adm_vref", verify_ref_bytes(current)) && ctx_buf(c, "ref_first", (size_t)refine_first_cap() * 4) &&
               pinned_report(c, PINNED_VERIFY) && ctx_buf(c, "adm_xi8_spec", (size_t)T * ld * ld) &&
               ctx_buf(c, "adm_ci32_spec", (size_t)T * ld * ld * 4) && ctx_buf(c, "adm_vref2", verify_ref_bytes(current));
    }
    bool check_applies(bool confirming, bool from_packed) const {
        return guess_applies(confirming) && verify_applies(confirming, from_packed) && lab.sym && mode == SDPSR_SQUARE_I8 &&
               square_check_supports(n, current, 2, T) && !(c->opts.flags & SDPSR_FLAG_SQUARE_EVERY_VERDICT) &&
               (proj_dead || r == 0 || current <= (int64_t)verify_lds_cap());
    }
    bool checks_deferrable() const {
        return c->allow_deferred_verdict && c->pinned_small != nullptr && !tm.enabled && !(c->opts.flags & SDPSR_FLAG_CHECKS_IN_LOOP);
    }
    int check_round(const SigSource& qj, uint64_t key2, bool tail, Verdict* v) {
        SquareCheck q;
        q.n = n, q.d = current, q.G = 2, q.T = T;
        void* ws = ctx_buf(c, "adm_sqcheck", square_check_ws_bytes(n, current, 2, T));
        const uint32_t* first = (const uint32_t*)ctx_buf(c, "ref_first", (size_t)refine_first_cap() * 4);
        uint32_t* hv = pinned_report(c, PINNED_VERIFY);
        uint32_t* hv2 = pinned_report(c, PINNED_SPECULATIVE);
        if (!ws || !first || !hv || !hv2) return SDPSR_OUT_OF_MEMORY;
        const bool defer = c->allow_deferred_verdict && c->pinned_small != nullptr;
        if (defer) hv = c->pinned_small + PINNED_SMALL_DEFERRED_VERIFY.first, hv2 = c->pinned_small + PINNED_SMALL_DEFERRED_SPECULATIVE.first;
        square_check_ws_carve(q, ws);
        q.key[0] = key2, q.key[1] = next_key(c);
        q.Lp = lab.Lp, q.Lp8 = lab.shadow(), q.first_idx = first, q.Lfull = lab.full_from_gather();
        q.flag[0] = hv, q.flag[1] = hv2;
        const bool proj_verify = qj.kind == SIG_JOINT_I32 && r >= 1;
        if (tail && !defer) return ctx_fail(c, SDPSR_BAD_STATE, "admissible_subspace: check segment asked for where the verdicts are read in the loop");
        if (tail) {
            *(volatile uint32_t*)hv = DEFERRED_NEVER_RAN;
            *(volatile uint32_t*)hv2 = DEFERRED_NEVER_RAN;
            const bool on_record = rec_full != nullptr && c->initial_guess_pending && q.Lfull == lab.L;
            if (!on_record) launch_square_check_ref_and_pass(s, q);
            DeferredTail& t = c->deferred_tail;
            if (t.next == t.count) t.next = t.count = 0;
            if (t.count >= DEFERRED_SEGMENTS) return ctx_fail(c, SDPSR_BAD_STATE, "admissible_subspace: no room for the round's check segment");
            DeferredSegment& g = t.seg[t.count++] = DeferredSegment{};
            g.kind = DEFERRED_CHECK, g.q = qj, g.n = n, g.d = current, g.first = first, g.flag = hv;
            g.Lp = lab.Lp, g.Lp8 = lab.shadow();
            g.proj_coef = !proj_dead, g.partial = partial, g.coef = coef, g.nblk = nblk;
            g.proj_verify = proj_verify;
            g.verdict = true, g.sq = q;
            ++c->check_stats.registered;
            if (on_record) {
                DeferredSegment& g0 = t.seg[t.next];
                if (&g0 != &g && g0.pair && g0.n == g.n && g0.Lp == g.Lp && g0.Lp8 == g.Lp8 && g0.first == g.first) {
                    g.pair = true, g.a = g0.a, g.b = g0.b, g.pair_d = g0.pair_d, g.pair_flag = g0.pair_flag;
                    g0.pair = false;
                }
                g0.sq_pass = true, g0.sq = q;
                c->labels_on_record = rec_full;
            }
        } else {
            *(volatile uint32_t*)hv = 0u;
            *(volatile uint32_t*)hv2 = 0u;
            launch_square_check_ref_and_pass(s, q);
            if (proj_verify) launch_verify_projection(s, qj, current, first, hv);
            launch_square_check_verdict(s, q);
        }
        c->squares_launched += 2, ++c->squares_speculative, ++c->square_checks;
        if (defer) {
            c->deferred_verdict = true;
            HIP_TRY(c, hipGetLastError());
            v->unchanged = v->spec_confirmed = true;
            return SDPSR_OK;
        }
        HIP_TRY(c, ctx_sync_stream(c, s));
        HIP_TRY(c, hipGetLastError());
        v->unchanged = hv[0] == 0;
        v->spec_confirmed = v->unchanged && hv2[0] == 0;
        if (!v->spec_confirmed) --c->stream_counter;
        if (!v->unchanged) {
            ++c->square_check_fallbacks;
            --c->squares_launched;
            launch_square(true, key2, Xp, Cp, current);
        }
        return SDPSR_OK;
    }
    int verify_round(const SigSource& qj, bool confirming, bool from_packed, bool tail, Verdict* v) {
        if (!verify_applies(confirming, from_packed)) return SDPSR_OK;
        SigSource qv = qj;
        if (confirming) qv.kind = SIG_CHAN_I32;
        void* vref = ctx_buf(c, "adm_vref", verify_ref_bytes(current));
        const uint32_t* first = (const uint32_t*)ctx_buf(c, "ref_first", (size_t)refine_first_cap() * 4);
        uint32_t* hv = pinned_report(c, PINNED_VERIFY);
        uint32_t* hv2 = pinned_report(c, PINNED_SPECULATIVE);
        if (!vref || !first || !hv) return SDPSR_OUT_OF_MEMORY;
        const bool guess = guess_applies(confirming);
        const bool defer = guess && c->allow_deferred_verdict && c->pinned_small != nullptr;
        if (defer) hv = c->pinned_small + PINNED_SMALL_DEFERRED_VERIFY.first, hv2 = c->pinned_small + PINNED_SMALL_DEFERRED_SPECULATIVE.first;
        if (tail) {
            int8_t* Xs = (int8_t*)ctx_buf(c, "adm_xi8_spec", (size_t)T * ld * ld);
            int32_t* Cs = (int32_t*)ctx_buf(c, "adm_ci32_spec", (size_t)T * ld * ld * 4);
            void* vref2 = ctx_buf(c, "adm_vref2", verify_ref_bytes(current));
            if (!Xs || !Cs || !vref2) return SDPSR_OUT_OF_MEMORY;
            launch_square(true, next_key(c), Xs, Cs, current, true, true);
            DeferredTail& t = c->deferred_tail;
            t.ld = ld, t.d = current, t.T = T, t.zero_flag = zero_flag, t.first = first;
            t.seg[0] = t.seg[1] = DeferredSegment{};
            t.seg[0].X = (const int8_t*)Xp, t.seg[0].C = (int32_t*)Cp, t.seg[0].q = qv, t.seg[0].vref = vref, t.seg[0].flag = hv, t.seg[0].speculative = false;
            t.seg[1].X = Xs, t.seg[1].C = Cs, t.seg[1].q = qj, t.seg[1].vref = vref2, t.seg[1].flag = hv2, t.seg[1].speculative = true;
            t.seg[1].q.kind = SIG_CHAN_I32, t.seg[1].q.C = Cs;
            *(volatile uint32_t*)hv = DEFERRED_NEVER_RAN;
            *(volatile uint32_t*)hv2 = DEFERRED_NEVER_RAN;
// ... 169 lines not shown
        return SDPSR_OK;
    }
    int initial_partition(const double* dCL, const double* dX0, int hint, const InitialRecord* guess, int64_t* d) {
        SigSource q;
        q.kind = SIG_PAIR, q.sig = sig, q.a = dCL, q.b = dX0;
        if (!((hint & 2) && lab.Lp && len < (int64_t(1) << 32))) return lab.refine_full(q, d, true);
        q.n = n, q.packed = 1, lab.sym = 1;
        initial_packed = true;
        const uint8_t* Lp8 = guess ? lab.Lp8 : nullptr;
        if (guess) {
            uint32_t* over = c->pinned_small + PINNED_SMALL_DEFERRED_NARROW.first;
            *(volatile uint32_t*)over = 0u;
            if (Lp8 && !(guess->narrow && guess->Lp8 == Lp8)) {
                launch_labels_narrow(s, n * (n + 1) / 2, lab.Lp, lab.Lp8, 8, over, c->num_cus);
                ++c->label_narrowings;
            }
        }
        bool pair_registered = false;
        if (guess && checks_deferrable() && !(c->opts.flags & SDPSR_FLAG_SQUARE_EVERY_VERDICT) && n < (int64_t(1) << 31) && guess->d0 >= 1 &&
            guess->d0 <= (int64_t)verify_lds_cap()) {
            flush_deferred_tail(c);
            DeferredTail& t = c->deferred_tail;
            DeferredSegment& g = t.seg[0] = DeferredSegment{};
            g.kind = DEFERRED_CHECK, g.pair = true, g.n = n, g.a = dCL, g.b = dX0, g.Lp = lab.Lp, g.Lp8 = Lp8, g.pair_d = guess->d0, g.first = guess->first;
            g.pair_flag = c->pinned_small + PINNED_SMALL_DEFERRED_INITIAL.first;
            *(volatile uint32_t*)g.pair_flag = DEFERRED_NEVER_RAN;
            t.next = 0, t.count = 1;
            ++c->check_stats.registered;
            pair_registered = true;
        }
        if (guess && (pair_registered || launch_verify_pair(s, n, dCL, dX0, lab.Lp, guess->d0, guess->first, c->pinned_small + PINNED_SMALL_DEFERRED_INITIAL.first, Lp8))) {
            c->initial_guess_pending = true;
            ++c->initial_guesses;
            HIP_TRY(c, hipGetLastError());
            *d = guess->d0;
            lab.packed_refined();
            lab.shadow_current();
            c->table_log2_hint = refine_table_hint(n * (n + 1) / 2, (uint64_t)guess->d0);
            return SDPSR_OK;
        }
        return lab.refine_packed(q, d);
    }
    int initial_guess_settled() {
        if (!c->initial_guess_pending) return SDPSR_OK;
        flush_deferred_tail(c);
        HIP_TRY(c, ctx_sync_stream(c, s));
        HIP_TRY(c, hipGetLastError());
        if (initial_guess_violated(c) != 0) return STATUS_REPEAT_REDUCTION;
        c->initial_guess_pending = false;
        return SDPSR_OK;
    }
    bool initial_packed = false;
    const uint32_t* rec_full = nullptr;
    int square_buffers() {
        static const struct { const char *x, *c; size_t xb, cb; } B[] = {{"adm_xi8", "adm_ci32", 1, 4}, {"adm_xf32", "adm_cf32", 4, 4}, {"adm_xf64", "adm_cf64", 8, 8}};
        if (mode < SDPSR_SQUARE_I8 || mode > SDPSR_SQUARE_F64) return ctx_fail(c, SDPSR_BAD_ARGUMENT, "unknown square_mode");
        const size_t e = (size_t)T * ld * ld;
        Xp = ctx_buf(c, B[mode - SDPSR_SQUARE_I8].x, e * B[mode - SDPSR_SQUARE_I8].xb);
        Cp = ctx_buf(c, B[mode - SDPSR_SQUARE_I8].c, e * B[mode - SDPSR_SQUARE_I8].cb);
        if (mode == SDPSR_SQUARE_F32) {
            vmax = std::min(127, (int)std::floor(std::sqrt(16777216.0 / (double)n)));
            if (vmax < 1) return ctx_fail(c, SDPSR_BAD_ARGUMENT, "n too large for the exact fp32 square");
        }
        if (mode == SDPSR_SQUARE_F64 && !(Y = (double*)ctx_buf(c, "adm_y", (size_t)len * 8))) return SDPSR_OUT_OF_MEMORY;
        return (Xp && Cp) ? SDPSR_OK : SDPSR_OUT_OF_MEMORY;
    }
};
}

namespace sdpsr {
void flush_deferred_tail(sdpsr_ctx* c, int max_segments, bool in_ride) {
    DeferredTail& t = c->deferred_tail;
    if (!in_ride && t.next < t.count) deferred_window_close(c);
    for (; max_segments > 0 && t.next < t.count; --max_segments, ++t.next) {
        const DeferredSegment& g = t.seg[t.next];
        if (g.kind == DEFERRED_CHECK) {
            if (g.sq_pass) launch_square_check_ref_and_pass(c->stream, g.sq);
            if (g.pair) launch_verify_pair(c->stream, g.n, g.a, g.b, g.Lp, g.pair_d, g.first, g.pair_flag, g.Lp8);
            if (g.verdict) {
                *(volatile uint32_t*)g.sq.flag[0] = 0u;
                *(volatile uint32_t*)g.sq.flag[1] = 0u;
                if (g.proj_coef) launch_proj_coef_lower(c->stream, g.n, g.q.r, g.q.U, g.Lp, 1, g.q.key, g.partial, g.nblk, g.coef, g.Lp8);
                if (g.proj_verify) launch_verify_projection(c->stream, g.q, g.d, g.first, g.flag);
                launch_square_check_verdict(c->stream, g.sq);
            }
            ++(in_ride ? c->check_stats.in_ride : c->check_stats.outside_ride);
            continue;
        }
        launch_gemm_tn_i8_sym(c->stream, t.ld, t.ld, g.X, t.ld, g.C, t.ld, t.T, t.ld * t.ld, t.ld * t.ld, t.zero_flag, c->num_cus, c->opts.square_kernel);
        ++c->squares_launched;
        if (g.speculative) ++c->squares_speculative;
        launch_verify_no_split(c->stream, g.q, t.d, t.first, g.vref, g.flag);
    }
}

int admissible_subspace_impl(sdpsr_ctx* c, int64_t n, const double* CL, const double* X0L, const double* U, int64_t r, double atol,
                             uint32_t* P_out, int64_t* dim_out, int32_t* iters_out, double* phase_ms, int mem, int mem_out,
                             bool final_sync, int* labels_sym_out) {
    CHECK_CTX(c);
    const int hint = c->hint_symmetric_basis;
    c->hint_symmetric_basis = 0;
    c->hint_used = hint;
    c->adm_dims.clear();
    const InitialRecord rec = c->initial_record;
    c->initial_record = InitialRecord{};
    if (!CL || !X0L || !P_out || !dim_out || n < 1 || r < 0 || (r > 0 && !U) || !(atol > 0))
        return ctx_fail(c, SDPSR_BAD_ARGUMENT, "bad arguments");
    const int64_t len = n * n;
    int st = check_len(c, len);
    if (st) return st;
    hipStream_t s = c->stream;
    PhaseTimer tm(c, phase_ms != nullptr);
    TotalEvents ev_total(phase_ms != nullptr, s);

    c->table_log2_hint = 12;
    Loop lp(c, tm);
    lp.n = n, lp.len = len, lp.ld = round_up(n, 128), lp.r = r, lp.atol = atol;
    lp.early_ok = !(c->opts.flags & SDPSR_FLAG_WAIT_FOR_EVERY_VERDICT);
    const double* dCL = in_dev(c, "adm_cl", CL, len, mem, &st);
    const double* dX0 = in_dev(c, "adm_x0", X0L, len, mem, &st);
    lp.dU = in_dev(c, "adm_u", U, (size_t)len * std::max<int64_t>(r, 1), mem, &st);
    lp.lab.L = out_dev(c, "adm_labels", P_out, len, mem_out, &st);
    lp.sig = (uint64_t*)ctx_buf(c, "sig", len * 8);
    lp.partial = (double*)ctx_buf(c, "proj_partial", (size_t)2 * std::max<int64_t>(r, 1) * lp.nblk * 8);
    lp.coef = (double*)ctx_buf(c, "proj_coef", (size_t)2 * std::max<int64_t>(r, 1) * 8);
    lp.symflag = (uint32_t*)ctx_buf(c, "adm_symflag", 64);
    if (st || !lp.sig || !lp.partial || !lp.coef || !lp.symflag) return st ? st : SDPSR_OUT_OF_MEMORY;
    if (!c->symflag_zero) HIP_TRY(c, hipMemsetAsync(lp.symflag, 0, 64, s));
    c->symflag_zero = true;
    lp.zero_flag = lp.symflag + 8;
    lp.mode = c->opts.square_mode, lp.T = (lp.mode == SDPSR_SQUARE_F64) ? 1 : c->opts.channels;
    st = lp.square_buffers();
    if (st) return st;
    lp.scale = round_scale(c, atol);
    lp.int_mode = (lp.mode == SDPSR_SQUARE_I8 || lp.mode == SDPSR_SQUARE_F32);
    lp.lab.Lp = lp.int_mode ? (uint32_t*)ctx_buf(c, "adm_lpacked", (size_t)(n * (n + 1) / 2) * 4) : nullptr;
    if (lp.int_mode && !lp.lab.Lp) return SDPSR_OUT_OF_MEMORY;
    lp.keep_packed = lp.mode == SDPSR_SQUARE_I8 && (lp.T == 1 || lp.T == 2 || lp.T == 4) && !(c->opts.flags & SDPSR_FLAG_UNPACK_EVERY_STEP);
    lp.lab.init(c, n, lp.symflag, lp.keep_packed, lp.early_ok);

    const bool first_joint = !(c->opts.flags & (SDPSR_FLAG_SEPARATE_REFINEMENTS | SDPSR_FLAG_NO_VERIFY_SHORTCUT)) && lp.keep_packed && (lp.T == 2 || lp.T == 4) &&
                             (r == 0 || (hint & 1)) && r <= 4 && len < (int64_t(1) << 32) && c->opts.max_iters >= 1;
    const bool guess_initial = c->allow_deferred_verdict && c->pinned_small && lp.early_ok && c->predict_closed && c->predict_n == n && (hint & 2) && first_joint &&
                               rec.valid && rec.n == n && rec.Lp == lp.lab.Lp && rec.sym == 1 && rec.d0 >= 1 && rec.d0 <= (int64_t)verify_lds_cap() &&
                               c->first_idx_labels == lp.lab.Lp && rec.first == (const uint32_t*)ctx_buf(c, "ref_first", (size_t)refine_first_cap() * 4);
    if (dbg_on() && c->allow_deferred_verdict && !guess_initial)
        fprintf(stderr, "[sdpsr] loop: initial partition not guessed (predicted closed %d at n %lld, hint %d, joint first iteration %d, record %d: n %lld, d0 %lld, "
                        "labels %d, representatives of them %d)\n", (int)c->predict_closed, (long long)c->predict_n, hint, (int)first_joint, (int)rec.valid,
                (long long)rec.n, (long long)rec.d0, (int)(rec.Lp == lp.lab.Lp), (int)(c->first_idx_labels == lp.lab.Lp));
    if (guess_initial && rec.d0 <= 255 && !(c->opts.flags & SDPSR_FLAG_WIDE_LOOP_LABELS))
        lp.lab.Lp8 = (uint8_t*)ctx_buf(c, "adm_lpacked8", (size_t)(n * (n + 1) / 2));
    const bool record_labels = c->record_labels_allowed && c->allow_deferred_verdict && c->pinned_small && !tm.enabled && first_joint && (hint & 2) &&
                               lp.mode == SDPSR_SQUARE_I8 && !(c->opts.flags & (SDPSR_FLAG_CHECKS_IN_LOOP | SDPSR_FLAG_SQUARE_EVERY_VERDICT));
    if (guess_initial && record_labels && rec.Lfull && rec.Lfull == (const uint32_t*)ctx_buf(c, "adm_lfull_rec", (size_t)len * 4)) lp.rec_full = rec.Lfull;
    int64_t d = 0;
    tm.begin(SDPSR_T_REFINE);
    st = lp.initial_partition(dCL, dX0, hint, guess_initial ? &rec : nullptr, &d);
    tm.end();
    if (st) return st;
    tm.collect();
    c->adm_dims.assign(1, d);
    if (label_overflows(c, (uint64_t)d)) return label_overflow_fail(c, "admissible_subspace: dim(S)", (uint64_t)d);
    lp.basis_sym = (r == 0) || (hint & 1) != 0, lp.probe_pending = !lp.basis_sym;

    const int64_t maximal = (len + n) / 2;
    lp.current = d, lp.confirm_left = c->opts.confirm_rounds;
    bool converged = lp.current >= maximal;
    const bool separate = (c->opts.flags & SDPSR_FLAG_SEPARATE_REFINEMENTS) != 0;
    while (lp.current < maximal) {
        if (lp.it >= c->opts.max_iters) break;
        ++lp.it;
        tm.begin(SDPSR_T_PROJECT);
        lp.key = next_key(c);
        lp.packed_proj = lp.int_mode && lp.lab.sym && lp.basis_sym && r <= 4 && len < (int64_t(1) << 32);
        const bool joint = !separate && lp.packed_proj && lp.keep_packed && (lp.T == 2 || lp.T == 4) && c->table_log2_hint < 21;
        int64_t dn = lp.current;
        st = joint ? lp.joint_iteration(&dn) : lp.separate_iteration(&dn);
        if (st) return st;
        c->adm_dims.push_back(dn);
        if (label_overflows(c, (uint64_t)dn)) return label_overflow_fail(c, "admissible_subspace: dim(S)", (uint64_t)dn);
        if (dn == lp.current) {
            converged = true;
            break;
        }
        lp.confirm_left = c->opts.confirm_rounds;
        lp.current = dn;
        if (lp.current >= maximal) converged = true;
    }
    lp.lab.need_full();
    HIP_TRY(c, hipGetLastError());
    c->predict_closed = converged && lp.it == 1 && c->adm_dims.size() == 2 && c->adm_dims[0] == c->adm_dims[1];
    c->predict_n = n;
    if (converged && lp.initial_packed && c->first_idx_labels == lp.lab.Lp && c->adm_dims[0] >= 1 && c->adm_dims[0] <= (int64_t)verify_lds_cap() &&
        std::all_of(c->adm_dims.begin(), c->adm_dims.end(), [&](int64_t x) { return x == c->adm_dims[0]; })) {
        const uint32_t* lfull = guess_initial ? rec.Lfull : nullptr;
        if (!lfull && record_labels && lp.lab.sym && square_check_supports(n, c->adm_dims[0], 2, lp.T)) {
            uint32_t* copy = (uint32_t*)ctx_buf(c, "adm_lfull_rec", (size_t)len * 4);
            if (copy && hipMemcpyAsync(copy, lp.lab.L, (size_t)len * 4, hipMemcpyDeviceToDevice, s) == hipSuccess) lfull = copy;
            else (void)hipGetLastError();
        }
        InitialRecord& ir = c->initial_record;
        ir.first = (const uint32_t*)ctx_buf(c, "ref_first", (size_t)refine_first_cap() * 4);
        ir.Lfull = lfull;
        ir.n = n, ir.d0 = c->adm_dims[0], ir.Lp = lp.lab.Lp, ir.sym = lp.lab.sym;
        ir.narrow = lp.lab.narrow(), ir.Lp8 = ir.narrow ? lp.lab.Lp8 : nullptr;
        ir.valid = ir.first != nullptr;
    } else {
        c->labels_on_record = nullptr;
    }
    *dim_out = lp.current;
    if (iters_out) *iters_out = lp.it;
    if (labels_sym_out) *labels_sym_out = lp.lab.sym;
    if (final_sync || mem_out != SDPSR_MEM_DEVICE) {
        st = out_finish(c, P_out, lp.lab.L, len, mem_out);
        if (st) return st;
    }
    if (phase_ms) {
        const float ms = ev_total.stop(s);
        tm.collect();
        for (int i = 0; i < SDPSR_T_COUNT; ++i) phase_ms[i] = tm.acc[i];
        phase_ms[SDPSR_T_TOTAL] = ms;
    }
    if (!converged) return ctx_fail(c, SDPSR_NOT_CONVERGED, "max_iters reached");
    return SDPSR_OK;
}
}

extern "C" {
int sdpsr_admissible_subspace(sdpsr_ctx* c, int64_t n, const double* CL, const double* X0L,
                              const double* U, int64_t r, double atol, uint32_t* P_out,
                              int64_t* dim_out, int32_t* iters_out, double* phase_ms, int mem) {
    if (!c || c->label_width == 32 || !P_out || !dim_out || n < 1)
        return admissible_subspace_impl(c, n, CL, X0L, U, r, atol, P_out, dim_out, iters_out, phase_ms, mem, mem, true, nullptr);
    CHECK_CTX(c);
    uint32_t* L = (uint32_t*)ctx_buf(c, "adm_labels", (size_t)n * n * 4);
    if (!L) return SDPSR_OUT_OF_MEMORY;
    const int st = admissible_subspace_impl(c, n, CL, X0L, U, r, atol, L, dim_out, iters_out, phase_ms, mem, SDPSR_MEM_DEVICE, true, nullptr);
    if (st && st != SDPSR_NOT_CONVERGED) return st;
    if (label_width_overflows(c, (uint64_t)*dim_out)) return label_width_fail(c, "admissible_subspace", (uint64_t)*dim_out);
    const int st_out = labels_out_finish(c, P_out, L, (size_t)n * n, mem);
    return st_out ? st_out : st;
}

int sdpsr_desymmetrize(sdpsr_ctx* c, int64_t n, uint32_t* P, int64_t* dim, int32_t* iters, int mem) {
    CHECK_CTX(c);
    if (!P || !dim || n < 1) return ctx_fail(c, SDPSR_BAD_ARGUMENT, "bad arguments");
    const int64_t len = n * n;
    int st = check_len(c, len);
    if (st) return st;
    uint32_t* L = (mem == SDPSR_MEM_DEVICE && c->label_width == 32) ? P : (uint32_t*)labels_in_dev(c, "adm_labels", (const uint32_t*)P, len, mem, &st);
    if (st) return st;
    st = desymmetrize_device(c, n, L, dim, iters);
    if (st) return st;
    if (label_width_overflows(c, (uint64_t)*dim)) return label_width_fail(c, "desymmetrize", (uint64_t)*dim);
    return labels_out_finish(c, P, L, len, mem);
}
}

int sdpsr::desymmetrize_device(sdpsr_ctx* c, int64_t n, uint32_t* L, int64_t* dim, int32_t* iters) {
    const int64_t len = n * n;
    int st = SDPSR_OK;
// ... 36 lines not shown
```

### sdpsymmetryreduction.jl_amd/csrc/prof/prof.cpp

```cpp
#include <algorithm>
#include <cmath>
#include <complex>
#include <cstdio>
#include <cstdlib>
#include <cstring>
#include <chrono>
#include <functional>
#include <numeric>

#include <rocblas/rocblas.h>
#include <rocsolver/rocsolver.h>

#include "../host_internal.h"
#include "../../../include/sdpsr_prof.h"

using namespace sdpsr;

namespace sdpsr {
void launch_fill_test_sig(hipStream_t s, int64_t len, int64_t nclasses, uint64_t* sig);
void launch_clock_sampler(hipStream_t s, long long* buf, int ns, const unsigned* flag, long long max_ticks, int* count);
void launch_wall_marker(hipStream_t s, long long* out);
bool launch_band_chase(hipStream_t s, int n, int b, double* A, int64_t ld, unsigned* progress, unsigned* abort_flag, double* d, double* e, int max_wgs);
void launch_band_panel_split(hipStream_t s, int64_t m, int b, double* P, int64_t ldp, double* V, int64_t ldv);
}
// ... 297 lines not shown
extern "C" int sdpsr_profile_gather_packed_w(sdpsr_ctx* c, int64_t n, int T, int64_t d, uint64_t key, int width, const uint32_t* Lp_host,
                                             int8_t* X_plain, int8_t* X_writing, uint32_t* L_inout, int64_t guard) {
    return prof_gather_packed(c, n, T, d, key, width, Lp_host, nullptr, X_plain, X_writing, nullptr, L_inout, guard);
}
extern "C" int sdpsr_profile_verify(sdpsr_ctx* c, int64_t n, int T, int64_t d, int mode, const uint32_t* Lp_host, const uint32_t* first_idx_host,
                                    const int32_t* C_host, const double* U_host, double coef, uint64_t key, double atol, uint32_t* out) {
    if (mode == 2) return prof_basis_constant(c, n, 1, d, Lp_host, first_idx_host, U_host, atol, out);
    if (mode != 0 && mode != 1) return c ? ctx_fail(c, SDPSR_BAD_ARGUMENT, "bad arguments") : SDPSR_BAD_ARGUMENT;
    return prof_verify(c, n, T, d, mode == 1 ? 1 : -1, 32, Lp_host, first_idx_host, C_host, U_host, &coef, key, atol, out);
}
extern "C" int sdpsr_profile_verify_w(sdpsr_ctx* c, int64_t n, int T, int64_t d, int r, int width, const uint32_t* Lp_host,
                                      const uint32_t* first_idx_host, const int32_t* C_host, const double* U_host, const double* coef_host,
                                      uint64_t key, double atol, uint32_t* out) {
    return prof_verify(c, n, T, d, r, width, Lp_host, first_idx_host, C_host, U_host, coef_host, key, atol, out);
}
extern "C" int sdpsr_profile_basis_constant(sdpsr_ctx* c, int64_t n, int r, int64_t d, const uint32_t* Lp_host, const uint32_t* first_idx_host,
                                            const double* U_host, double atol, uint32_t* out) {
    return prof_basis_constant(c, n, r, d, Lp_host, first_idx_host, U_host, atol, out);
}
extern "C" int sdpsr_profile_verify_pair(sdpsr_ctx* c, int64_t n, int64_t d, const uint32_t* Lp_host, const uint32_t* first_idx_host,
                                         const double* a_host, const double* b_host, uint32_t* out) {
    return prof_verify_pair(c, n, d, 32, Lp_host, first_idx_host, a_host, b_host, out);
}
extern "C" int sdpsr_profile_verify_pair_w(sdpsr_ctx* c, int64_t n, int64_t d, int width, const uint32_t* Lp_host, const uint32_t* first_idx_host,
                                           const double* a_host, const double* b_host, uint32_t* out) {
    return prof_verify_pair(c, n, d, width, Lp_host, first_idx_host, a_host, b_host, out);
}

extern "C" int sdpsr_profile_square_checks(sdpsr_ctx* c, int32_t restart, uint64_t* out) {
    CHECK_CTX(c);
    if (!out || restart < 0 || restart > (int32_t)c->batch_children.size()) return ctx_fail(c, SDPSR_BAD_ARGUMENT, "bad arguments");
    const sdpsr_ctx* ci = restart == 0 ? c : c->batch_children[restart - 1];
    out[0] = ci->square_checks;
    out[1] = ci->square_check_fallbacks;
    return SDPSR_OK;
}

extern "C" int sdpsr_profile_deferred_checks(sdpsr_ctx* c, int32_t restart, uint64_t* out) {
    CHECK_CTX(c);
    if (!out || restart < 0 || restart > (int32_t)c->batch_children.size()) return ctx_fail(c, SDPSR_BAD_ARGUMENT, "bad arguments");
    const DeferredCheckStats& t = (restart == 0 ? c : c->batch_children[restart - 1])->check_stats;
    out[0] = t.registered, out[1] = t.in_ride, out[2] = t.outside_ride;
    out[3] = t.window_ns[0], out[4] = t.window_count[0], out[5] = t.window_ns[1], out[6] = t.window_count[1];
    out[7] = t.voided[0], out[8] = t.voided[1], out[9] = t.voided[2];
    return SDPSR_OK;
}
extern "C" int sdpsr_profile_recorded_labels(sdpsr_ctx* c, int32_t restart, uint64_t* out) {
    const int st = sdpsr_profile_deferred_checks(c, restart, out);
    if (st) return st;
    out[10] = (restart == 0 ? c : c->batch_children[restart - 1])->check_stats.on_record;
    return SDPSR_OK;
}

extern "C" int sdpsr_profile_square_check(sdpsr_ctx* c, int64_t n, int64_t d, int G, int T, const uint64_t* keys, int width, int write_full,
                                          const uint32_t* Lp_host, const uint32_t* first_idx_host, uint8_t* ws_inout, uint64_t* layout,
                                          uint32_t* verdicts_out, uint32_t* L_inout, int64_t guard) {
    CHECK_CTX(c);
    constexpr size_t gap = 64;
    if (!layout || !square_check_supports(n, d, G, T) || n > 8192 || (width != 8 && width != 32) || guard < 0 || guard > (int64_t(1) << 20))
        return ctx_fail(c, SDPSR_BAD_ARGUMENT, "bad arguments");
    SquareCheck q;
    q.n = n, q.d = d, q.G = G, q.T = T;
    const size_t bytes = square_check_ws_carve(q, nullptr, gap);
    void* ws = ctx_buf(c, "prof_sqcheck", bytes);
    if (!ws) return SDPSR_OUT_OF_MEMORY;
    square_check_ws_carve(q, ws, gap);
    const void* parts[7] = {q.c, q.part_x, q.part_c, q.y, q.w, q.esum, q.bits};
    for (int k = 0; k < 7; ++k) layout[k] = (uint64_t)((const char*)parts[k] - (const char*)ws);
    layout[7] = bytes;
    if (!ws_inout) return SDPSR_OK;
    if (!keys || !Lp_host || !first_idx_host || !verdicts_out || (write_full && !L_inout)) return ctx_fail(c, SDPSR_BAD_ARGUMENT, "null pointer");
    hipStream_t s = c->stream;
    uint32_t* Lw = write_full ? (uint32_t*)ctx_buf(c, "prof_lwritten", (size_t)(n * n + guard) * 4) : nullptr;
    uint32_t* flag1 = pinned_report(c, PINNED_SPECULATIVE);
    if ((write_full && !Lw) || !flag1) return SDPSR_OUT_OF_MEMORY;
    ProfClasses p;
    const int st = prof_classes_up(c, n, d, width, Lp_host, first_idx_host, &p);
    if (st) return st;
    HIP_TRY(c, hipMemcpyAsync(ws, ws_inout, bytes, hipMemcpyHostToDevice, s));
    if (write_full) HIP_TRY(c, hipMemcpyAsync(Lw, L_inout, (size_t)(n * n + guard) * 4, hipMemcpyHostToDevice, s));
    for (int g = 0; g < G; ++g) q.key[g] = keys[g];
    q.Lp = p.Lp, q.Lp8 = p.Lp8, q.first_idx = p.first, q.Lfull = Lw;
    q.flag[0] = p.flag, q.flag[1] = flag1;
    *(volatile uint32_t*)q.flag[0] = 0u;
    *(volatile uint32_t*)q.flag[1] = 0u;
    launch_square_check_ref_and_pass(s, q);
    launch_square_check_verdict(s, q);
    HIP_TRY(c, hipMemcpyAsync(ws_inout, ws, bytes, hipMemcpyDeviceToHost, s));
    if (write_full) HIP_TRY(c, hipMemcpyAsync(L_inout, Lw, (size_t)(n * n + guard) * 4, hipMemcpyDeviceToHost, s));
    HIP_TRY(c, hipStreamSynchronize(s));
    HIP_TRY(c, hipGetLastError());
    verdicts_out[0] = ((const volatile uint32_t*)q.flag[0])[0];
    verdicts_out[1] = ((const volatile uint32_t*)q.flag[1])[0];
    return SDPSR_OK;
}

extern "C" int sdpsr_profile_proj_coef_lower(sdpsr_ctx* c, int64_t n, int64_t r, uint64_t key, int width, const uint32_t* Lp_host,
                                             const double* U_host, double* partial_out, double* coef_out) {
    CHECK_CTX(c);
    if (!Lp_host || !U_host || !partial_out || !coef_out || n < 1 || n > 8192 || r < 1 || r > 4) return ctx_fail(c, SDPSR_BAD_ARGUMENT, "bad arguments");
    constexpr int nblk = 2048;
    hipStream_t s = c->stream;
    const int64_t np = n * (n + 1) / 2;
    uint32_t* Lp = (uint32_t*)ctx_buf(c, "prof_lp", (size_t)np * 4);
    double* Ud = (double*)ctx_buf(c, "prof_vu", (size_t)(n * n + 1) * 4 * 8);
    double* partial = (double*)ctx_buf(c, "prof_partial", (size_t)(r * nblk + r) * 8);
// ... 235 lines not shown
}

extern "C" int sdpsr_profile_class_sums2(sdpsr_ctx* c, int64_t n, int64_t d, uint32_t first, int plain, const uint32_t* L_host, const double* X_host,
                                         double* Y_inout, int64_t guard, int32_t* report) {
    CHECK_CTX(c);
    if (!L_host || !X_host || !Y_inout || !report || n < 1 || n > MK_MAX_N || d < 1 || d > 4000 || first < 1 || (plain != 0 && plain != 1) ||
        (plain && first != 1) || guard < 0 || guard > MK_MAX_GUARD)
        return ctx_fail(c, SDPSR_BAD_ARGUMENT, "class_sums2: bad arguments");
    if ((size_t)64 * ((d + 1) | 1) * 16 > 150 * 1024) return ctx_fail(c, SDPSR_BAD_ARGUMENT, "class_sums2: no instance for this many classes");
    if (plain && !mk_labels_ok(L_host, (size_t)n * n, d)) return ctx_fail(c, SDPSR_BAD_ARGUMENT, "class_sums2: a label exceeds d");
    hipStream_t s = c->stream;
    const size_t yn = (size_t)(2 * n * d + guard);
    uint32_t* Lb = (uint32_t*)ctx_buf(c, "prof_l", (size_t)n * n * 4);
    double* X = (double*)ctx_buf(c, "prof_mk_a", (size_t)2 * n * 8);
    double* Y = (double*)ctx_buf(c, "prof_mk_c", yn * 8);
    if (!Lb || !X || !Y) return SDPSR_OUT_OF_MEMORY;
    HIP_TRY(c, hipMemcpyAsync(Lb, L_host, (size_t)n * n * 4, hipMemcpyHostToDevice, s));
    HIP_TRY(c, hipMemcpyAsync(X, X_host, (size_t)2 * n * 8, hipMemcpyHostToDevice, s));
    HIP_TRY(c, hipMemcpyAsync(Y, Y_inout, yn * 8, hipMemcpyHostToDevice, s));
    const int W = launch_class_sums_pair(s, n, d, first, plain != 0, Lb, X, Y);
    HIP_TRY(c, hipMemcpyAsync(Y_inout, Y, yn * 8, hipMemcpyDeviceToHost, s));
    HIP_TRY(c, hipStreamSynchronize(s));
    HIP_TRY(c, hipGetLastError());
    if (!W) return ctx_fail(c, SDPSR_BAD_ARGUMENT, "class_sums2: no instance for this many classes");
    report[0] = W;
    return SDPSR_OK;
}

extern "C" int sdpsr_profile_class_sums(sdpsr_ctx* c, int64_t n, int64_t d, int64_t ldo, const uint32_t* L_host, const double* x_host,
                                        double* out_inout, int64_t guard, int32_t* report) {
    CHECK_CTX(c);
    if (!L_host || !x_host || !out_inout || !report || n < 1 || n > MK_MAX_N || d < 1 || d > 4000 || ldo < n || ldo > MK_MAX_LD || guard < 0 ||
        guard > MK_MAX_GUARD)
        return ctx_fail(c, SDPSR_BAD_ARGUMENT, "class_sums: bad arguments");
    if (!mk_labels_ok(L_host, (size_t)n * n, d)) return ctx_fail(c, SDPSR_BAD_ARGUMENT, "class_sums: a label exceeds d");
    const bool table = class_sums_supports(n, d, n + 1);
    report[0] = class_sums_supports(n, d, ldo) ? 1 : 0;
    report[1] = table ? 1 : 0;
    if (!report[0]) return SDPSR_OK;
    if (!table && !basis_image_two_stage_fits(n, d, 1)) return ctx_fail(c, SDPSR_BAD_ARGUMENT, "class_sums: the fallback does not take this shape");
    hipStream_t s = c->stream;
    const size_t on = (size_t)(ldo * d + guard);
    uint32_t* Lb = (uint32_t*)ctx_buf(c, "prof_l", (size_t)n * n * 4);
    double* x = (double*)ctx_buf(c, "prof_mk_a", (size_t)n * 8);
    double* out = (double*)ctx_buf(c, "prof_mk_c", on * 8);
    if (!Lb || !x || !out) return SDPSR_OUT_OF_MEMORY;
    HIP_TRY(c, hipMemcpyAsync(Lb, L_host, (size_t)n * n * 4, hipMemcpyHostToDevice, s));
    HIP_TRY(c, hipMemcpyAsync(x, x_host, (size_t)n * 8, hipMemcpyHostToDevice, s));
    HIP_TRY(c, hipMemcpyAsync(out, out_inout, on * 8, hipMemcpyHostToDevice, s));
    launch_class_sums(s, n, d, Lb, x, out, ldo, 1);
    HIP_TRY(c, hipMemcpyAsync(out_inout, out, on * 8, hipMemcpyDeviceToHost, s));
    HIP_TRY(c, hipStreamSynchronize(s));
    HIP_TRY(c, hipGetLastError());
    return SDPSR_OK;
}

extern "C" int sdpsr_profile_symmetrize(sdpsr_ctx* c, int64_t m, int64_t ld, double* B_inout, int64_t guard) {
    CHECK_CTX(c);
    if (!B_inout || m < 1 || m > 1024 || ld < m || ld > 2048 || guard < 0 || guard > MK_MAX_GUARD) return ctx_fail(c, SDPSR_BAD_ARGUMENT, "symmetrize: bad arguments");
    hipStream_t s = c->stream;
    const size_t bn = (size_t)(ld * m + guard);
    double* B = (double*)ctx_buf(c, "prof_mk_c", bn * 8);
    if (!B) return SDPSR_OUT_OF_MEMORY;
    HIP_TRY(c, hipMemcpyAsync(B, B_inout, bn * 8, hipMemcpyHostToDevice, s));
    launch_symmetrize(s, m, ld, B);
    HIP_TRY(c, hipMemcpyAsync(B_inout, B, bn * 8, hipMemcpyDeviceToHost, s));
    HIP_TRY(c, hipStreamSynchronize(s));
    HIP_TRY(c, hipGetLastError());
    return SDPSR_OK;
}

extern "C" int sdpsr_profile_extract_symmetric(sdpsr_ctx* c, int64_t m, int64_t mp, int64_t lds, const double* src_host, double* dst_inout, int64_t guard) {
    CHECK_CTX(c);
    if (!src_host || !dst_inout || m < 1 || mp < m || mp > 1024 || lds < m || lds > 2048 || guard < 0 || guard > MK_MAX_GUARD)
        return ctx_fail(c, SDPSR_BAD_ARGUMENT, "extract_symmetric: bad arguments");
    hipStream_t s = c->stream;
    const size_t dn = (size_t)(mp * mp + guard);
    double* src = (double*)ctx_buf(c, "prof_mk_a", (size_t)lds * m * 8);
    double* dst = (double*)ctx_buf(c, "prof_mk_c", dn * 8);
    if (!src || !dst) return SDPSR_OUT_OF_MEMORY;
    HIP_TRY(c, hipMemcpyAsync(src, src_host, (size_t)lds * m * 8, hipMemcpyHostToDevice, s));
    HIP_TRY(c, hipMemcpyAsync(dst, dst_inout, dn * 8, hipMemcpyHostToDevice, s));
    launch_extract_symmetric(s, m, mp, src, lds, dst);
    HIP_TRY(c, hipMemcpyAsync(dst_inout, dst, dn * 8, hipMemcpyDeviceToHost, s));
    HIP_TRY(c, hipStreamSynchronize(s));
    HIP_TRY(c, hipGetLastError());
    return SDPSR_OK;
}

extern "C" int sdpsr_profile_normalize_columns(sdpsr_ctx* c, int64_t n, int64_t ldx, int64_t hstride, int64_t nruns, const double* X_host,
                                               double* H_inout, double* norm_inout, int64_t guard) {
    CHECK_CTX(c);
    if (!X_host || !H_inout || !norm_inout || n < 1 || n > MK_MAX_N || ldx < n || ldx > MK_MAX_LD || nruns < 1 || nruns > 64 ||
        (nruns > 1 && hstride < n) || hstride < 0 || hstride > 4 * MK_MAX_LD || guard < 0 || guard > MK_MAX_GUARD)
        return ctx_fail(c, SDPSR_BAD_ARGUMENT, "normalize_columns: bad arguments");
    hipStream_t s = c->stream;
    const size_t hn = (size_t)(hstride * (nruns - 1) + n + guard), nn = (size_t)(nruns + guard);
    double* X = (double*)ctx_buf(c, "prof_mk_a", (size_t)ldx * nruns * 8);
    double* H = (double*)ctx_buf(c, "prof_mk_c", hn * 8);
    double* nrm = (double*)ctx_buf(c, "prof_mk_b", nn * 8);
    if (!X || !H || !nrm) return SDPSR_OUT_OF_MEMORY;
    HIP_TRY(c, hipMemcpyAsync(X, X_host, (size_t)ldx * nruns * 8, hipMemcpyHostToDevice, s));
    HIP_TRY(c, hipMemcpyAsync(H, H_inout, hn * 8, hipMemcpyHostToDevice, s));
    HIP_TRY(c, hipMemcpyAsync(nrm, norm_inout, nn * 8, hipMemcpyHostToDevice, s));
    launch_normalize_columns(s, n, ldx, H, hstride, X, ldx, (int)nruns, nrm);
    HIP_TRY(c, hipMemcpyAsync(H_inout, H, hn * 8, hipMemcpyDeviceToHost, s));
// ... 815 lines not shown
```

### sdpsymmetryreduction.jl_amd/csrc/reduce.cpp

```cpp
#include <algorithm>
#include <cstring>
#include <new>

#include "host_internal.h"

using namespace sdpsr;

namespace sdpsr {
int jordan_reduce_impl(sdpsr_ctx* c, int64_t n, const double* CL, const double* X0L, const double* U, int64_t r, double atol, double epsilon,
                       uint32_t* P_out, int64_t* dim_out, int32_t* iters_out, int32_t* nblocks, int64_t* sum_sq, int64_t* sum_s, double* blks,
                       int64_t blks_capacity, double* Q_hat, int64_t qhat_capacity, double* phase_ms, int mem_in, int mem_out) {
    const int mem = mem_out;
    CHECK_CTX(c);
    if (!dim_out || n < 1 || !(epsilon > 0) || blks_capacity < 0 || qhat_capacity < 0 || (blks_capacity > 0 && !blks) ||
        (qhat_capacity > 0 && !Q_hat))
        return ctx_fail(c, SDPSR_BAD_ARGUMENT, "bad arguments");
    const int64_t len = n * n;
    int st = check_len(c, len);
    if (st) return st;
    hipStream_t s = c->stream;
    const uint64_t stream_at_entry = c->stream_counter;
    const int hint_at_entry = c->hint_symmetric_basis;
    const bool in_place = mem == SDPSR_MEM_DEVICE && P_out != nullptr && c->label_width == 32;
    uint32_t* L = in_place ? P_out : (uint32_t*)ctx_buf(c, "bd_labels", (size_t)len * 4);
    if (!L) return SDPSR_OUT_OF_MEMORY;
    c->bd_valid = false;
    c->bd_q_valid = false;
    c->bd_qrm_current = false;
    c->bd_labels_ext = nullptr;
    double pm_a[SDPSR_T_COUNT] = {}, pm_b[SDPSR_T_COUNT] = {}, pm_i[SDPSR_T_COUNT] = {};
    int labels_sym = 0;
    c->deferred_verdict = false;
    c->initial_guess_pending = false;
    struct DropTail {
        sdpsr_ctx* c;
        ~DropTail() {
            c->deferred_tail.count = c->deferred_tail.next = 0;
            c->check_stats.window_open = -1;
        }
    } drop_tail{c};
    c->check_stats.window_open = -1;
    auto repeat_without_guesses = [&](uint32_t dv, uint32_t dv_spec, uint32_t dv_init) -> int {
        c->predict_closed = false;
        c->initial_record = InitialRecord{};
        if (dv_init != 0) ++c->initial_guesses_violated;
        c->check_stats.voided[0] = dv, c->check_stats.voided[1] = dv_spec, c->check_stats.voided[2] = dv_init;
        if (dbg_on())
            fprintf(stderr, "[sdpsr] jordan_reduce: %s%s%s (deferred verdicts: verify %u, speculative %u, initial partition %u): reduction repeated\n",
                    dv_init != 0 ? "the initial partition was not the recorded one" : "", dv_init != 0 && (dv != 0 || dv_spec != 0) ? "; " : "",
                    dv != 0 ? "the input was not closed after all" : (dv_spec != 0 ? "the confirm round found a split" : ""), dv, dv_spec, dv_init);
        c->stream_counter = stream_at_entry;
        c->hint_symmetric_basis = hint_at_entry;
        if (mem_in != SDPSR_MEM_DEVICE) {
            CL = (const double*)ctx_buf(c, "adm_cl", (size_t)len * 8);
            X0L = (const double*)ctx_buf(c, "adm_x0", (size_t)len * 8);
            if (U) U = (const double*)ctx_buf(c, "adm_u", (size_t)len * std::max<int64_t>(r, 1) * 8);
            if (!CL || !X0L || (r > 0 && !U)) return SDPSR_OUT_OF_MEMORY;
            mem_in = SDPSR_MEM_DEVICE;
        }
        return jordan_reduce_impl(c, n, CL, X0L, U, r, atol, epsilon, P_out, dim_out, iters_out, nblocks, sum_sq, sum_s, blks, blks_capacity, Q_hat,
                                  qhat_capacity, phase_ms, mem_in, mem_out);
    };
    auto leave = [&](int st_err) -> int {
        if (!c->initial_guess_pending) return st_err;
        c->initial_guess_pending = false;
        c->deferred_verdict = false;
        flush_deferred_tail(c);
        if (ctx_sync_stream(c, s) != hipSuccess) return st_err == STATUS_REPEAT_REDUCTION ? ctx_fail(c, SDPSR_HIP_ERROR, "hipStreamSynchronize failed") : st_err;
        const uint32_t dv_init = initial_guess_violated(c);
        if (dv_init != 0) return repeat_without_guesses(0, 0, dv_init);
        return st_err == STATUS_REPEAT_REDUCTION ? ctx_fail(c, SDPSR_BAD_STATE, "jordan_reduce: a repeat was asked for without a violated verdict") : st_err;
    };
    c->allow_deferred_verdict = !(c->opts.flags & SDPSR_FLAG_WAIT_FOR_EVERY_VERDICT);
    c->record_labels_allowed = in_place && !phase_ms && !(c->opts.flags & SDPSR_FLAG_LABELS_BEFORE_BLOCKDIAG);
    c->labels_on_record = nullptr;
    st = admissible_subspace_impl(c, n, CL, X0L, U, r, atol, L, dim_out, iters_out, phase_ms ? pm_a : nullptr, mem_in, SDPSR_MEM_DEVICE,
                                  false, &labels_sym);
    c->allow_deferred_verdict = false;
    c->record_labels_allowed = false;
    const uint32_t* Lbd = c->labels_on_record ? c->labels_on_record : L;
    c->labels_on_record = nullptr;
    const int st_loop = st;
    if (st && st != SDPSR_NOT_CONVERGED) return leave(st);
    const bool overflow = P_out && label_width_overflows(c, (uint64_t)*dim_out);
    if (P_out && !in_place && !overflow) {
        st = labels_deliver(c, P_out, L, (size_t)len, mem);
        if (st) return leave(st);
    }
    const int64_t d = *dim_out;
    int32_t nb = 0;
    int64_t S = 0, S1 = 0;
    if (!overflow && Lbd != L) ++c->check_stats.on_record;
    st = overflow ? SDPSR_OK
                  : block_diagonalize_impl(c, n, Lbd, d, epsilon, &nb, &S, &S1, phase_ms ? pm_b : nullptr, SDPSR_MEM_DEVICE, labels_sym != 0,
                                           false, in_place);
    flush_deferred_tail(c);
    if (nblocks) *nblocks = nb;
    if (sum_sq) *sum_sq = S;
    if (sum_s) *sum_s = S1;
    bool images_done = false;
    if (st == SDPSR_OK && !overflow && blks && d * S <= blks_capacity && (!Q_hat || n * S1 <= qhat_capacity)) {
        st = sdpsr_block_images(c, blks, (Q_hat && n * S1 <= qhat_capacity) ? Q_hat : nullptr, phase_ms ? pm_i : nullptr, mem);
        images_done = st == SDPSR_OK;
    }
    if (in_place) {
        struct Forget {
            sdpsr_ctx* c;
            bool ok = false;
            ~Forget() {
                c->bd_labels_ext = nullptr;
                c->bd_trusted_symmetric = nullptr;
                if (!ok) c->bd_valid = false;
            }
        } forget{c};
        if (!images_done && c->bd_valid) {
            uint32_t* keep = (uint32_t*)ctx_buf(c, "bd_labels", (size_t)len * 4);
            if (!keep) return leave(SDPSR_OUT_OF_MEMORY);
            const hipError_t ek = hipMemcpyAsync(keep, P_out, (size_t)len * 4, hipMemcpyDeviceToDevice, s);
            if (ek != hipSuccess) return leave(ctx_fail(c, SDPSR_HIP_ERROR, std::string("hipMemcpyAsync: ") + hipGetErrorString(ek)));
        } else if (images_done) {
            c->bd_valid = false;
        }
        forget.ok = true;
    }
    if (!images_done) {
        flush_deferred_tail(c);
        const hipError_t e = ctx_sync_stream(c, s);
        if (e != hipSuccess && st == SDPSR_OK) st = ctx_fail(c, SDPSR_HIP_ERROR, std::string("hipStreamSynchronize: ") + hipGetErrorString(e));
    }
    if (c->deferred_verdict || c->initial_guess_pending) {
        const volatile uint32_t* ps = c->pinned_small;
        const uint32_t dv = c->deferred_verdict ? ps[PINNED_SMALL_DEFERRED_VERIFY.first] : 0u;
        const uint32_t dv_spec = c->deferred_verdict ? ps[PINNED_SMALL_DEFERRED_SPECULATIVE.first] : 0u;
        const uint32_t dv_init = c->initial_guess_pending ? initial_guess_violated(c) : 0u;
        c->deferred_verdict = false;
        c->initial_guess_pending = false;
        if (dv != 0 || dv_spec != 0 || dv_init != 0) {
            const int st2 = repeat_without_guesses(dv, dv_spec, dv_init);
            if (phase_ms)
                for (int i = 0; i < SDPSR_T_COUNT; ++i) phase_ms[i] += pm_a[i] + pm_b[i] + pm_i[i];
            return st2;
        }
    }
    if (phase_ms) {
        for (int i = 0; i < SDPSR_T_COUNT; ++i) phase_ms[i] = pm_a[i] + pm_b[i] + pm_i[i];
    }
    if (overflow && st == SDPSR_OK) return label_width_fail(c, "jordan_reduce: admissible_subspace", (uint64_t)d);
    if (st == SDPSR_OK && P_out && !in_place) st = labels_delivered(c);
    return st ? st : st_loop;
}
}

extern "C" int sdpsr_jordan_reduce(sdpsr_ctx* c, int64_t n, const double* CL, const double* X0L, const double* U, int64_t r,
                                   double atol, double epsilon, uint32_t* P_out, int64_t* dim_out, int32_t* iters_out,
                                   int32_t* nblocks, int64_t* sum_sq, int64_t* sum_s, double* blks, int64_t blks_capacity,
                                   double* Q_hat, int64_t qhat_capacity, double* phase_ms, int mem) {
    return jordan_reduce_impl(c, n, CL, X0L, U, r, atol, epsilon, P_out, dim_out, iters_out, nblocks, sum_sq, sum_s, blks, blks_capacity, Q_hat,
                              qhat_capacity, phase_ms, mem, mem);
}

extern "C" int sdpsr_problem_create(sdpsr_ctx* c, int64_t n, const double* CL, const double* X0L, const double* U, int64_t r, int hint, int mem,
                                    sdpsr_problem** out) {
    CHECK_CTX(c);
// ... 59 lines not shown
```

### sdpsymmetryreduction.jl_amd/csrc/sdpsr_internal.h

```cpp
#pragma once
#include <hip/hip_runtime.h>
#include <stdint.h>
#include <stddef.h>

#include <map>
#include <functional>
#include <string>
#include <string_view>
#include <vector>

#include "../../include/sdpsr.h"
#include "sdpsr_hash.h"

namespace sdpsr { struct SytrdGraphCache; }

struct DevBuf {
    void* p = nullptr;
    size_t bytes = 0;
};

namespace sdpsr {
enum { SIG_ARRAY = 0, SIG_PAIR = 1, SIG_PROJ = 2, SIG_CHAN_I32 = 3, SIG_CHAN_F32 = 4, SIG_JOINT_I32 = 5 };
struct SigSource {
    int kind = SIG_ARRAY;
// ... 21 lines not shown
    const uint32_t* Lp = nullptr;
    const uint8_t* Lp8 = nullptr;
    const uint32_t* first_idx = nullptr;
    uint32_t* Lfull = nullptr;
    uint32_t* flag[2] = {nullptr, nullptr};
    int32_t *c = nullptr, *part_x = nullptr;
    int64_t *part_c = nullptr, *y = nullptr, *w = nullptr;
    uint64_t* esum = nullptr;
    uint32_t* bits = nullptr;
};

enum { DEFERRED_SQUARE = 0, DEFERRED_CHECK = 1 };
struct DeferredSegment {
    int kind = DEFERRED_SQUARE;
    const int8_t* X = nullptr;
    int32_t* C = nullptr;
    SigSource q;
    void* vref = nullptr;
    uint32_t* flag = nullptr;
    bool speculative = false;
    bool sq_pass = false;
    bool pair = false;
    int64_t pair_d = 0;
    uint32_t* pair_flag = nullptr;
    const double *a = nullptr, *b = nullptr;
    const uint32_t* Lp = nullptr;
    const uint8_t* Lp8 = nullptr;
    int64_t n = 0, d = 0;
    const uint32_t* first = nullptr;
    bool proj_coef = false;
    double* partial = nullptr;
    double* coef = nullptr;
    int nblk = 0;
    bool proj_verify = false;
    bool verdict = false;
    SquareCheck sq;
};
constexpr int DEFERRED_SEGMENTS = 2;
struct DeferredTail {
    DeferredSegment seg[DEFERRED_SEGMENTS];
    int count = 0, next = 0;
    int64_t ld = 0, d = 0;
    int T = 0;
    const uint32_t* zero_flag = nullptr;
    const uint32_t* first = nullptr;
};
struct DeferredCheckStats {
    uint64_t registered = 0, in_ride = 0, outside_ride = 0;
    uint64_t window_ns[2] = {0, 0}, window_count[2] = {0, 0};
    int window_open = -1;
    uint64_t window_t0 = 0;
    uint32_t voided[3] = {0, 0, 0};
    uint64_t on_record = 0;
};
constexpr uint32_t DEFERRED_NEVER_RAN = 0xDEFE44EDu;
struct InitialRecord {
    bool valid = false;
    int64_t n = 0, d0 = 0;
    const uint32_t *Lp = nullptr, *first = nullptr;
    int sym = 0;
    bool narrow = false;
    const uint8_t* Lp8 = nullptr;
    const uint32_t* Lfull = nullptr;
};
constexpr int STATUS_REPEAT_REDUCTION = -0x5250;
}

struct sdpsr_ctx {
    int device = 0;
    int num_cus = 256;
    uint64_t seed = 0;
    uint64_t stream_counter = 0;
    sdpsr_opts opts{};
    int label_width = 32;
    hipStream_t stream = nullptr;
    hipStream_t side_stream = nullptr;
    hipEvent_t ev_fork = nullptr, ev_join = nullptr, ev_wait = nullptr;
    hipEvent_t ev_bt_fork = nullptr, ev_bt_join = nullptr;
    hipStream_t main_shadow = nullptr;
    bool own_stream = false;
    std::string err;
    double dbg_last_ms = 0;
    std::map<std::string, DevBuf, std::less<>> bufs;
    void* pinned = nullptr;
    size_t pinned_bytes = 0;
    uint32_t* pinned_small = nullptr;
    void* h2d_ring = nullptr;
    int h2d_ring_next = 0;
    void* rocblas = nullptr;
    sdpsr::SytrdGraphCache* sytrd_graphs = nullptr;
    int64_t bd_n = 0, bd_d = 0;
    std::vector<int32_t> bd_sizes;
    int64_t bd_sum_s = 0, bd_sum_sq = 0;
    bool bd_valid = false;
    int64_t bdc_n = 0, bdc_d = 0, bdc_sum_s = 0, bdc_sum_sq = 0;
    std::vector<int32_t> bdc_sizes;
    bool bdc_valid = false;
    uint32_t bd_sym_epoch = 0;
    const uint32_t* bd_sym_labels = nullptr;
    const uint32_t* bd_labels_ext = nullptr;
    const uint32_t* bd_trusted_symmetric = nullptr;
    uint32_t epoch_counter = 0;
    const uint32_t* first_idx_labels = nullptr;
    int hint_symmetric_basis = 0;
    std::vector<int64_t> adm_dims;
    bool bd_q_valid = false;
    bool bd_labels_owned = false;
    bool bd_qrm_current = false;
    int table_log2_hint = 12;
    uint64_t refine_passes = 0;
    hipEvent_t ev[2 * SDPSR_T_COUNT] = {};
    void (*yield_fn)(void*) = nullptr;
    void* yield_arg = nullptr;
    std::vector<sdpsr_ctx*> batch_children;
    uint64_t h2d_bytes = 0, d2h_bytes = 0;
    bool predict_closed = false;
    int64_t predict_n = 0;
    uint64_t squares_launched = 0, squares_speculative = 0;
    uint64_t square_checks = 0, square_check_fallbacks = 0;
    int hint_used = 0;
    uint64_t host_waits = 0;
    uint32_t report_seq = 0;
    bool allow_deferred_verdict = false;
    bool deferred_verdict = false;
    sdpsr::DeferredTail deferred_tail;
    sdpsr::DeferredCheckStats check_stats;
    sdpsr::InitialRecord initial_record;
    bool initial_guess_pending = false;
    bool record_labels_allowed = false;
    const uint32_t* labels_on_record = nullptr;
    uint64_t initial_guesses = 0, initial_guesses_violated = 0;
    uint64_t label_narrowings = 0;
    bool symflag_zero = false;
};

struct sdpsr_problem {
    int device = 0;
    int64_t n = 0, r = 0;
    double *CL = nullptr, *X0 = nullptr, *U = nullptr;
    int hint = 0;
};

struct sdpsr_sparse {
    int device = 0;
    int64_t len = 0, m = 0, nnz = 0;
    int64_t* rowptr = nullptr;
    uint32_t* col = nullptr;
    double* val = nullptr;
    int rows_symmetric = 0;
};

struct sdpsr_blockop {
    int device = 0;
    int64_t d = 0, sum_sq = 0, nnz_full = 0;
    std::vector<int32_t> sizes;
    void* by_class = nullptr;
    void* by_pos = nullptr;
};

struct BlocksSyevJob {
    int64_t zoff, woff;
    int32_t n, pad;
};

inline hipError_t ctx_sync_stream(sdpsr_ctx* c, hipStream_t s) {
    if (c) ++c->host_waits;
    if (!c || !c->yield_fn) return hipStreamSynchronize(s);
    const hipError_t before = hipPeekAtLastError();
    for (;;) {
        const hipError_t e = hipStreamQuery(s);
        if (e != hipErrorNotReady) {
            if (hipPeekAtLastError() == hipErrorNotReady) (void)hipGetLastError();
            if (e == hipSuccess && before != hipSuccess && before != hipErrorNotReady) return before;
            return e;
        }
        c->yield_fn(c->yield_arg);
    }
}

inline hipError_t ctx_wait_word(sdpsr_ctx* c, hipStream_t s, const volatile uint32_t* w, uint32_t seq) {
    ++c->host_waits;
    const hipError_t before = hipPeekAtLastError();
    bool queried = false;
// ... 241 lines not shown
void launch_gemm_tn_i8_sym(hipStream_t s, int64_t n, int64_t k, const int8_t* X, int64_t ldx, int32_t* C, int64_t ldc,
                           int batch, int64_t strideX, int64_t strideC, const uint32_t* nonsym_flag, int num_cus = 0,
                           int variant = 0);
bool launch_i8_symsquare(hipStream_t s, int64_t n, int64_t k, const int8_t* X, int64_t ldx, int32_t* C, int64_t ldc, int batch,
                         int64_t strideX, int64_t strideC, const uint32_t* nonsym_flag, int num_cus, int variant);
bool i8_symsquare_pays(int64_t n, int T, int num_cus);
bool gemm_sym_set_device_attributes();
void launch_gemm_tn_f32_sym(hipStream_t s, int64_t n, int64_t k, const float* X, int64_t ldx, float* C, int64_t ldc,
                            int batch, int64_t strideX, int64_t strideC, const uint32_t* nonsym_flag);
void launch_gemm_tn_i8(hipStream_t s, int64_t m, int64_t n, int64_t k, const int8_t* A,
                       int64_t lda, const int8_t* B, int64_t ldb, int32_t* C, int64_t ldc,
                       int batch, int64_t strideA, int64_t strideB, int64_t strideC);
void launch_gemm_tn_f32(hipStream_t s, int64_t m, int64_t n, int64_t k, const float* A,
                        int64_t lda, const float* B, int64_t ldb, float* C, int64_t ldc,
                        int batch, int64_t strideA, int64_t strideB, int64_t strideC);
void launch_gemm_tn_f64(hipStream_t s, int64_t m, int64_t n, int64_t k, const double* A,
                        int64_t lda, const double* B, int64_t ldb, double* C, int64_t ldc,
                        int batch, int64_t strideA, int64_t strideB, int64_t strideC);
void launch_gemm_tn_f64_sub(hipStream_t s, int64_t m, int64_t n, int64_t k, const double* A, int64_t lda, const double* B,
                            int64_t ldb, double* C, int64_t ldc);

void launch_small_qtaq_block_norms(hipStream_t s, int64_t n, int64_t ld, const double* A, const double* Q,
                                   const int32_t* space_of, int neig, unsigned long long* norms, double* Mout, double* Tout = nullptr);
size_t small_cluster_pack_bytes(int64_t n);
void launch_small_cluster_qtaq_block_norms(hipStream_t s, int64_t n, int64_t ld, const double* A, const double* Q,
                                           const double* evals, double atol, const int* einfo, char* pack, double* Tout);
void launch_coupling_symmetrize_minmax(hipStream_t s, int neig, unsigned long long* norms, const int32_t* dims, unsigned long long* stat);
void launch_coupling_count(hipStream_t s, int neig, const unsigned long long* norms, const double* edges17, unsigned long long* stat);
void launch_coupling_bits(hipStream_t s, int neig, const unsigned long long* norms, double thr, unsigned long long* bits);
void launch_block_norms(hipStream_t s, int64_t n, int64_t ld, const double* M,
                        const int32_t* space_of, int neig, unsigned long long* norms);
void launch_gemv_t(hipStream_t s, int64_t n, int64_t ld, const double* Q, int64_t col0,
                   int64_t m, const double* a, double* out);
void launch_gemv_n_scaled(hipStream_t s, int64_t n, int64_t ld, const double* Q, int64_t col0,
                          int64_t m, const double* w, const double* inv_norm, double* dst);
void launch_irreducible_pairs(hipStream_t s, int64_t n, int64_t ld, const double* Q, const double* Bf, int npairs,
                              int max_m2, const int32_t* desc, double* Qhat);
void launch_copy_cols(hipStream_t s, int64_t n, int64_t count, const int32_t* src_cols, const int32_t* dst_cols,
                      const double* src, int64_t ld_src, double* dst, int64_t ld_dst);
void launch_clamptol(hipStream_t s, int64_t len, double* a, double atol);
void launch_inv_norm(hipStream_t s, int64_t m, const double* v, double* out);

void launch_basis_image(hipStream_t s, int64_t n, int64_t d, int64_t S1, int64_t S,
                        const double* Qrm, const uint32_t* ent, const int64_t* class_ptr,
                        const int32_t* descA, const int32_t* descB, const int64_t* chunk_ptr,
                        int64_t nchunks_total, const int32_t* chunk_class,
                        const int64_t* chunk_begin, const int64_t* chunk_end, double* partial,
                        double* out, double atol);
bool basis_image_two_stage_fits(int64_t n, int64_t d, int64_t S1);
void launch_basis_image_outer(hipStream_t s, int64_t n, int64_t d, int64_t S1, int64_t S, int nblocks, int max_s,
                              const double* Qrm, const uint32_t* ent, const int64_t* cls_ptr,
                              const int32_t* blk_col, const int32_t* blk_size, const int64_t* blk_off, double atol,
                              double* out);
bool class_sums_supports(int64_t n, int64_t d, int64_t ldo);
void launch_class_sums(hipStream_t s, int64_t n, int64_t d, const uint32_t* L, const double* x, double* out, int64_t ldo, uint32_t first = 1);
int launch_class_sums_pair(hipStream_t s, int64_t n, int64_t d, uint32_t first, bool plain, const uint32_t* L, const double* X, double* Y);
void launch_basis_image_two_stage(hipStream_t s, int64_t n, int64_t d, uint32_t first, int64_t S1, int64_t S,
                                  const uint32_t* L, const double* Qrm, double* T, const int32_t* colA,
                                  const int32_t* colB, double atol, double* out);
size_t basis_image_commutative_workspace_doubles(int64_t n, int64_t d);
size_t basis_image_blocks_workspace_doubles(int64_t n, int64_t d);
bool launch_basis_image_blocks(hipStream_t s, int64_t n, int64_t d, uint32_t first, int64_t S1, int64_t S, int nblocks, const int32_t* blk_col, const int32_t* blk_size,
                               const int64_t* blk_off, const uint32_t* L, const double* Qrm, uint64_t key, int only, double atol, double tol, double* ws,
                               double* out, uint32_t* flag, bool plain = false);
bool launch_basis_image_fix_pair(hipStream_t s, int64_t n, int64_t d, uint32_t first, int64_t S1, const uint32_t* L, const double* Qrm, int k1, int k2,
                                 double atol, double* ws, double* out, bool plain = false);
bool launch_basis_image_commutative(hipStream_t s, int64_t n, int64_t d, uint32_t first, int64_t S1, const uint32_t* L, const double* Qrm, uint64_t key,
                                    double atol, double tol, double* ws, double* out, uint32_t* flag, bool plain = false);
void launch_transpose_to_rowmajor(hipStream_t s, int64_t n, int64_t S1, const double* Qcm,
                                  double* Qrm);
void launch_blocks_syev64(hipStream_t s, const BlocksSyevJob* jobs, int njac, int n1, int max_n, const double* Z, double* w, double* V,
                          int* flag);
size_t radix_sort_hist_words(int64_t len);
void launch_radix_sort_pairs(hipStream_t s, int64_t len, int bits, const uint32_t* keys, uint32_t* kA, uint32_t* kB, uint32_t* vA,
                             uint32_t* vB, uint32_t* hist, uint32_t first = 1, uint32_t cnt = 0xFFFFFFFFu);
int sort_entries_by_label(sdpsr_ctx* c, int64_t len, int64_t d, const uint32_t* L,
                          uint32_t** ent_out, std::vector<int64_t>& class_ptr_host, uint32_t first = 1);

int syev_device(sdpsr_ctx* c, int64_t n, double* A, int64_t lda, double* w, double* host_w = nullptr,
                const std::function<void()>* after_launch = nullptr, bool defer_readback = false);
void* ctx_pinned(sdpsr_ctx* c, size_t bytes);
void destroy_handle(sdpsr_ctx* c);

}
```

Measured before the change: 2501.

## Feed class sums from a lane-ordered byte copy of recorded labels

Adds a lane-ordered 8-bit copy of the recorded label matrix, produced while the admissible-subspace loop records its labels. Block diagonalization's class-sum kernel can read it instead of 32-bit labels, cutting label traffic by about four and allowing a deeper prefetch ring. The fetch pipeline is refactored into a generic BatchRing template. The byte path only applies when the recorded labels fit in 8 bits and the buffers match, and it adds one extra conversion pass and more bookkeeping state.

```diff
diff --git a/include/sdpsr.h b/include/sdpsr.h
--- a/include/sdpsr.h
+++ b/include/sdpsr.h
@@ -63,7 +63,8 @@
     SDPSR_FLAG_MODULE_SCRATCH_FILLS = 1u << 17,
     SDPSR_FLAG_SQUARE_EVERY_VERDICT = 1u << 18,
     SDPSR_FLAG_CHECKS_IN_LOOP = 1u << 19,
-    SDPSR_FLAG_LABELS_BEFORE_BLOCKDIAG = 1u << 20
+    SDPSR_FLAG_LABELS_BEFORE_BLOCKDIAG = 1u << 20,
+    SDPSR_FLAG_WIDE_BLOCKDIAG_LABELS = 1u << 21
 };
 
 typedef struct sdpsr_opts {
diff --git a/include/sdpsr_prof.h b/include/sdpsr_prof.h
--- a/include/sdpsr_prof.h
+++ b/include/sdpsr_prof.h
@@ -40,6 +40,7 @@
 int sdpsr_profile_square_checks(sdpsr_ctx* ctx, int32_t restart, uint64_t* out);
 int sdpsr_profile_deferred_checks(sdpsr_ctx* ctx, int32_t restart, uint64_t* out);
 int sdpsr_profile_recorded_labels(sdpsr_ctx* ctx, int32_t restart, uint64_t* out);
+int sdpsr_profile_record_bytes(sdpsr_ctx* ctx, int32_t restart, uint64_t* out);
 int sdpsr_profile_square_check(sdpsr_ctx* ctx, int64_t n, int64_t d, int G, int T, const uint64_t* keys, int width, int write_full,
                                const uint32_t* Lp_host, const uint32_t* first_idx_host, uint8_t* ws_inout, uint64_t* layout,
                                uint32_t* verdicts_out, uint32_t* L_inout, int64_t guard);
@@ -56,6 +57,9 @@
                                      int32_t* report);
 int sdpsr_profile_class_sums2(sdpsr_ctx* ctx, int64_t n, int64_t d, uint32_t first, int plain, const uint32_t* L_host, const double* X_host,
                               double* Y_inout, int64_t guard, int32_t* report);
+int sdpsr_profile_class_sums_bytes(sdpsr_ctx* ctx, int which, int64_t n, int64_t d, uint32_t first, int plain, int use_bytes,
+                                   const uint32_t* L_host, const double* X_host, double* Y_inout, int64_t guard, uint8_t* bytes_inout,
+                                   int32_t* report);
 int sdpsr_profile_class_sums(sdpsr_ctx* ctx, int64_t n, int64_t d, int64_t ldo, const uint32_t* L_host, const double* x_host,
                              double* out_inout, int64_t guard, int32_t* report);
 int sdpsr_profile_symmetrize(sdpsr_ctx* ctx, int64_t m, int64_t ld, double* B_inout, int64_t guard);
diff --git a/sdpsymmetryreduction.jl_amd/_lib.py b/sdpsymmetryreduction.jl_amd/_lib.py
--- a/sdpsymmetryreduction.jl_amd/_lib.py
+++ b/sdpsymmetryreduction.jl_amd/_lib.py
@@ -38,6 +38,7 @@
 FLAG_SQUARE_EVERY_VERDICT = 1 << 18
 FLAG_CHECKS_IN_LOOP = 1 << 19
 FLAG_LABELS_BEFORE_BLOCKDIAG = 1 << 20
+FLAG_WIDE_BLOCKDIAG_LABELS = 1 << 21
 BASIS_IMAGE_KERNELS = {"auto": 0, "two_stage": 1, "outer": 2, "chunk": 3}
 BI_ROUTE_COMMUTATIVE, BI_ROUTE_BLOCKS, BI_ROUTE_TWO_STAGE, BI_ROUTE_OUTER, BI_ROUTE_CHUNK = 1, 2, 3, 4, 5
 BI_ROUTE_REPAIRED, BI_ROUTE_SHORTCUT_REFUSED = 0x100, 0x200
@@ -250,6 +251,10 @@
     lib.sdpsr_profile_deferred_checks.argtypes = [vp, C.c_int32, C.POINTER(C.c_uint64)]
     lib.sdpsr_profile_recorded_labels.restype = C.c_int
     lib.sdpsr_profile_recorded_labels.argtypes = [vp, C.c_int32, C.POINTER(C.c_uint64)]
+    lib.sdpsr_profile_class_sums_bytes.restype = C.c_int
+    lib.sdpsr_profile_class_sums_bytes.argtypes = [vp, C.c_int, i64, i64, C.c_uint32, C.c_int, C.c_int, vp, vp, vp, i64, vp, C.POINTER(C.c_int32)]
+    lib.sdpsr_profile_record_bytes.restype = C.c_int
+    lib.sdpsr_profile_record_bytes.argtypes = [vp, C.c_int32, C.POINTER(C.c_uint64)]
     lib.sdpsr_profile_square_check.restype = C.c_int
     lib.sdpsr_profile_square_check.argtypes = [vp, i64, i64, C.c_int, C.c_int, vp, C.c_int, C.c_int, vp, vp, vp, vp, vp, vp, i64]
     lib.sdpsr_profile_proj_coef_lower.restype = C.c_int
diff --git a/sdpsymmetryreduction.jl_amd/csrc/blockdiag.cpp b/sdpsymmetryreduction.jl_amd/csrc/blockdiag.cpp
--- a/sdpsymmetryreduction.jl_amd/csrc/blockdiag.cpp
+++ b/sdpsymmetryreduction.jl_amd/csrc/blockdiag.cpp
@@ -10,7 +10,7 @@
 
 namespace sdpsr {
 static int keep_labels(sdpsr_ctx* c, int64_t n, const uint32_t* P, int mem, bool trusted_symmetric, bool in_place, bool labels_are_u32,
-                       uint32_t*& L) {
+                       const uint8_t* lane_bytes, uint32_t*& L) {
     hipStream_t s = c->stream;
     const int64_t len = n * n;
     int st = SDPSR_OK;
@@ -19,6 +19,7 @@
     L = in_place ? const_cast<uint32_t*>(P) : (uint32_t*)ctx_buf(c, "bd_labels", len * 4);
     if (!L) return SDPSR_OUT_OF_MEMORY;
     c->bd_labels_ext = in_place ? P : nullptr;
+    c->bd_lane_bytes = in_place ? lane_bytes : nullptr;
     c->bd_sym_labels = nullptr;
     c->bd_sym_epoch = 0;
     c->bd_trusted_symmetric = (trusted_symmetric && mem == SDPSR_MEM_DEVICE && P == L) ? L : nullptr;
@@ -55,7 +56,8 @@
 }
 
 int block_diagonalize_impl(sdpsr_ctx* c, int64_t n, const uint32_t* P, int64_t d, double epsilon, int32_t* nblocks, int64_t* sum_sq,
-                           int64_t* sum_s, double* phase_ms, int mem, bool trusted_symmetric, bool final_sync, bool in_place, bool labels_are_u32) {
+                           int64_t* sum_s, double* phase_ms, int mem, bool trusted_symmetric, bool final_sync, bool in_place, bool labels_are_u32,
+                           const uint8_t* lane_bytes) {
     CHECK_CTX(c);
     if (!P || n < 1 || d < 0 || !(epsilon > 0)) return ctx_fail(c, SDPSR_BAD_ARGUMENT, "bad arguments");
     const int64_t len = n * n;
@@ -68,7 +70,7 @@
     PhaseTimer tm(c, phase_ms != nullptr);
     TotalEvents ev_total(phase_ms != nullptr, s);
     uint32_t* L = nullptr;
-    st = keep_labels(c, n, P, mem, trusted_symmetric, in_place, labels_are_u32, L);
+    st = keep_labels(c, n, P, mem, trusted_symmetric, in_place, labels_are_u32, lane_bytes, L);
     if (st) return st;
     dbg_mark(c, "block_diagonalize: entered, labels copied");
     const double atol = epsilon;
diff --git a/sdpsymmetryreduction.jl_amd/csrc/compress.cpp b/sdpsymmetryreduction.jl_amd/csrc/compress.cpp
--- a/sdpsymmetryreduction.jl_amd/csrc/compress.cpp
+++ b/sdpsymmetryreduction.jl_amd/csrc/compress.cpp
@@ -213,7 +213,8 @@
         flush_deferred_tail(c);
         return SDPSR_OK;
     }
-    launch_class_sums(c->stream, n, d, L, W, W + (size_t)w * ld, ld);
+    const LaneBytes lb{L == c->bd_labels_ext ? c->bd_lane_bytes : nullptr, &c->check_stats.byte_class_sums};
+    launch_class_sums(c->stream, n, d, L, W, W + (size_t)w * ld, ld, 1, lb);
     window = 0;
     int got;
     live = (int)d;
diff --git a/sdpsymmetryreduction.jl_amd/csrc/ctx.cpp b/sdpsymmetryreduction.jl_amd/csrc/ctx.cpp
--- a/sdpsymmetryreduction.jl_amd/csrc/ctx.cpp
+++ b/sdpsymmetryreduction.jl_amd/csrc/ctx.cpp
@@ -22,7 +22,7 @@
     if (it != c->bufs.end() && it->second.bytes >= bytes) return it->second.p;
     DevBuf& b = it != c->bufs.end() ? it->second : c->bufs[std::string(name)];
     const std::string_view nm(name);
-    if (nm == "adm_lpacked" || nm == "adm_lpacked8" || nm == "ref_first" || nm == "adm_lfull_rec") c->initial_record = InitialRecord{};
+    if (nm == "adm_lpacked" || nm == "adm_lpacked8" || nm == "ref_first" || nm == "adm_lfull_rec" || nm == "adm_lfull8_rec") c->initial_record = InitialRecord{};
     if (nm == "adm_symflag") c->symflag_zero = false;
     if (nm == "bd_qhat" || nm == "bd_qrm") c->bd_qrm_current = false;
     if (b.p) {
diff --git a/sdpsymmetryreduction.jl_amd/csrc/host_internal.h b/sdpsymmetryreduction.jl_amd/csrc/host_internal.h
--- a/sdpsymmetryreduction.jl_amd/csrc/host_internal.h
+++ b/sdpsymmetryreduction.jl_amd/csrc/host_internal.h
@@ -265,7 +265,8 @@
                double* dCL, double* dX0, double* partial, int nblk, double* coef);
 int block_diagonalize_impl(sdpsr_ctx* c, int64_t n, const uint32_t* P, int64_t d, double epsilon, int32_t* nblocks, int64_t* sum_sq,
                            int64_t* sum_s, double* phase_ms, int mem, bool trusted_symmetric, bool final_sync, bool in_place = false,
-                           bool labels_are_u32 = true);
+                           bool labels_are_u32 = true,
+                           const uint8_t* lane_bytes = nullptr);
 
 struct EigInfo {
     std::vector<double> vals;
diff --git a/sdpsymmetryreduction.jl_amd/csrc/kernels_blockdiag.hip b/sdpsymmetryreduction.jl_amd/csrc/kernels_blockdiag.hip
--- a/sdpsymmetryreduction.jl_amd/csrc/kernels_blockdiag.hip
+++ b/sdpsymmetryreduction.jl_amd/csrc/kernels_blockdiag.hip
@@ -764,45 +764,129 @@
     return n <= 65535 && (2 * (d + 2) * 4 + n * 2) <= 60 * 1024 && d * n * S1 * 8 <= ((int64_t)4 << 30);
 }
 
+size_t lane_bytes_pitch(int64_t n) { return (size_t)512 * (size_t)((n + 511) / 512); }
 __global__ void __launch_bounds__(256)
-class_sums_small_d_kernel(int n, int d, uint32_t first, int tstride, const uint32_t* __restrict__ L, const double* __restrict__ x,
+lane_order_bytes_kernel(int n, int bpr, const uint32_t* __restrict__ L, uint2* __restrict__ B) {
+    const int64_t t = (int64_t)blockIdx.x * 256 + threadIdx.x;
+    if (t >= (int64_t)n * bpr * 64) return;
+    const int lane = (int)(t & 63);
+    const int64_t rb = t >> 6;
+    const int r = (int)(rb / bpr), bb = (int)(rb - (int64_t)r * bpr);
+    const uint32_t* col = L + (int64_t)r * n;
+    uint32_t w[2] = {0u, 0u};
+#pragma unroll
+    for (int u = 0; u < 8; ++u) {
+        const int c = bb * 512 + u * 64 + lane;
+        const uint32_t l = c < n ? (col[c] & 0xFFu) : 0u;
+        w[u >> 2] |= l << (8 * (u & 3));
+    }
+    B[t] = make_uint2(w[0], w[1]);
+}
+void launch_lane_order_bytes(hipStream_t s, int64_t n, const uint32_t* L, uint8_t* B) {
+    const int bpr = (int)((n + 511) / 512);
+    const int64_t threads = n * bpr * 64;
+    lane_order_bytes_kernel<<<(unsigned)((threads + 255) / 256), 256, 0, s>>>((int)n, bpr, L, reinterpret_cast<uint2*>(B));
+}
+
+template <bool BYTES>
+struct LabelBatch;
+template <>
+struct LabelBatch<false> {
+    uint32_t l[8];
+    __device__ __forceinline__ void load(const void* L, int n, int64_t, int r, int bb, int lane) {
+        const uint32_t* col = static_cast<const uint32_t*>(L) + (int64_t)r * n + bb * 512 + lane;
+        if ((bb + 1) * 512 <= n) {
+#pragma unroll
+            for (int u = 0; u < 8; ++u) l[u] = col[u * 64];
+        } else {
+#pragma unroll
+            for (int u = 0; u < 8; ++u) l[u] = col[bb * 512 + u * 64 + lane < n ? u * 64 : n - 1 - (bb * 512 + lane)];
+        }
+    }
+    __device__ __forceinline__ uint32_t label(int u) const { return l[u]; }
+};
+template <>
+struct LabelBatch<true> {
+    uint2 w;
+    __device__ __forceinline__ void load(const void* L, int, int64_t pitch, int r, int bb, int lane) {
+        w = *reinterpret_cast<const uint2*>(static_cast<const uint8_t*>(L) + (int64_t)r * pitch + bb * 512 + lane * 8);
+    }
+    __device__ __forceinline__ uint32_t label(int u) const { return ((u < 4 ? w.x : w.y) >> (8 * (u & 3))) & 0xFFu; }
+};
+struct NoBatch {};
+struct BatchCursor {
+    int rr = 0, bb = 0;
+    __device__ __forceinline__ void advance(int bpr) {
+        if (++bb == bpr) bb = 0, ++rr;
+    }
+};
+template <int NL, int NX, class LB, class XB>
+struct BatchRing {
+    static_assert(NL % NX == 0, "the buffers rotate by name");
+    LB q[NL];
+    XB x[NX];
+    BatchCursor cl, cx, cp;
+    template <class FL, class FX>
+    __device__ __forceinline__ void prime(int bpr, FL&& fetch_l, FX&& fetch_x) {
+#pragma unroll
+        for (int k = 0; k < NL - 1; ++k) fetch_l(cl, q[k]), cl.advance(bpr);
+#pragma unroll
+        for (int k = 0; k < NX - 1; ++k) fetch_x(cx, x[k]), cx.advance(bpr);
+    }
+    template <class FL, class FX, class P>
+    __device__ __forceinline__ void run(int rounds, int bpr, FL&& fetch_l, FX&& fetch_x, P&& process) {
+#pragma unroll 1
+        while (cp.rr < rounds) {
+#pragma unroll
+            for (int k = 0; k < NL; ++k) {
+                fetch_l(cl, q[(k + NL - 1) % NL]), cl.advance(bpr);
+                fetch_x(cx, x[(k + NX - 1) % NX]), cx.advance(bpr);
+                process(cp, q[k], x[k % NX]), cp.advance(bpr);
+            }
+        }
+    }
+};
+constexpr int CS_NBUF_U32 = 4, CS2_NBUF_U32 = 3;
+constexpr int CS_NBUF_BYTES = 16;
+
+template <bool BYTES>
+__global__ void __launch_bounds__(256)
+class_sums_small_d_kernel(int n, int d, uint32_t first, int tstride, const void* __restrict__ L, const double* __restrict__ x,
                           double* __restrict__ out, int64_t ldo) {
     extern __shared__ __attribute__((aligned(16))) double cs_smem[];
     double* sx = cs_smem;
-    const int lane = threadIdx.x & 63, wave = threadIdx.x >> 6;
+    const int lane = threadIdx.x & 63, wave = __builtin_amdgcn_readfirstlane(threadIdx.x >> 6);
     double* acc = cs_smem + n + (size_t)wave * 64 * tstride;
     double* mine = acc + (size_t)lane * tstride;
-    for (int c = threadIdx.x; c < n; c += 256) sx[c] = x[c];
-    __syncthreads();
     const int rows_per_round = gridDim.x * 4;
     const int bpr = (n + 511) / 512;
+    const int64_t pitch = (int64_t)bpr * 512;
     const int my_rows = (n - blockIdx.x * 4 + rows_per_round - 1) / rows_per_round;
-    const int total = my_rows * bpr;
-    auto fetch = [&](int bq, uint32_t (&lab)[8]) {
-        const int rr = bq / bpr, bb = bq - rr * bpr;
-        const int r = blockIdx.x * 4 + rr * rows_per_round + wave;
-        const uint32_t* col = L + (int64_t)((bq < total && r < n) ? r : 0) * n;
-#pragma unroll
-        for (int u = 0; u < 8; ++u) {
-            const int c = bb * 512 + u * 64 + lane;
-            lab[u] = col[c < n ? c : n - 1];
-        }
+    const int row0 = blockIdx.x * 4 + wave;
+    auto fetch = [&](const BatchCursor& c, LabelBatch<BYTES>& lab) {
+        const int r = row0 + c.rr * rows_per_round;
+        lab.load(L, n, pitch, (c.rr < my_rows && r < n) ? r : 0, c.bb, lane);
     };
-    auto process = [&](int bq, const uint32_t (&lab)[8]) {
-        if (bq >= total) return;
-        const int rr = bq / bpr, bb = bq - rr * bpr;
+    auto no_fetch = [](const BatchCursor&, NoBatch&) {};
+    auto process = [&](const BatchCursor& cur, const LabelBatch<BYTES>& lab, const NoBatch&) {
+        if (cur.rr >= my_rows) return;
+        const int rr = cur.rr, bb = cur.bb;
         if (bb == 0)
             for (int i = 0; i <= d; ++i) mine[i] = 0.0;
         double vv[8];
-#pragma unroll
-        for (int u = 0; u < 8; ++u) {
-            const int c = bb * 512 + u * 64 + lane;
-            vv[u] = c < n ? sx[c] : 0.0;
-        }
-#pragma unroll
-        for (int u = 0; u < 8; ++u) atomicAdd(&mine[window_label(lab[u], first, (uint32_t)d)], vv[u]);
+        const double* sxb = sx + bb * 512 + lane;
+        if ((bb + 1) * 512 <= n) {
+#pragma unroll
+            for (int u = 0; u < 8; ++u) vv[u] = sxb[u * 64];
+        } else {
+#pragma unroll
+            for (int u = 0; u < 8; ++u) vv[u] = bb * 512 + u * 64 + lane < n ? sxb[u * 64] : 0.0;
+        }
+#pragma unroll
+        for (int u = 0; u < 8; ++u)
+            atomicAdd(&mine[BYTES ? lab.label(u) : window_label(lab.label(u), first, (uint32_t)d)], vv[u]);
         if (bb == bpr - 1) {
-            const int r = blockIdx.x * 4 + rr * rows_per_round + wave;
+            const int r = row0 + rr * rows_per_round;
             __syncthreads();
             if (r < n)
                 for (int i = 1 + lane; i <= d; i += 64) {
@@ -813,21 +897,12 @@
             __syncthreads();
         }
     };
-    uint32_t qa[8], qb[8], qc[8], qd[8];
-    fetch(0, qa);
-    fetch(1, qb);
-    fetch(2, qc);
-#pragma unroll 1
-    for (int bq = 0; bq < total; bq += 4) {
-        fetch(bq + 3, qd);
-        process(bq, qa);
-        fetch(bq + 4, qa);
-        process(bq + 1, qb);
-        fetch(bq + 5, qb);
-        process(bq + 2, qc);
-        fetch(bq + 6, qc);
-        process(bq + 3, qd);
-    }
+    BatchRing<BYTES ? CS_NBUF_BYTES : CS_NBUF_U32, 1, LabelBatch<BYTES>, NoBatch> ring;
+    if (BYTES) ring.prime(bpr, fetch, no_fetch);
+    for (int c = threadIdx.x; c < n; c += 256) sx[c] = x[c];
+    __syncthreads();
+    if (!BYTES) ring.prime(bpr, fetch, no_fetch);
+    ring.run(my_rows, bpr, fetch, no_fetch, process);
 }
 
 __device__ __forceinline__ double bi_weight(uint64_t key, int k) {
@@ -876,48 +951,59 @@
     }
 }
 
+struct PairBatch {
+    double2 v[8];
+};
 template <int W, bool WIN>
 __global__ void __launch_bounds__(64 * W)
 class_sums2_kernel(int n, int d, uint32_t first, int tstride, const uint32_t* __restrict__ L, const double2* __restrict__ X,
                    double2* __restrict__ out) {
+    constexpr bool BYTES = false;
     extern __shared__ __attribute__((aligned(16))) double2 cs2_smem[];
-    const int lane = threadIdx.x & 63, wave = threadIdx.x >> 6;
+    const int lane = threadIdx.x & 63, wave = __builtin_amdgcn_readfirstlane(threadIdx.x >> 6);
     double2* acc = cs2_smem + (size_t)wave * 64 * tstride;
     double2* mine = acc + (size_t)lane * tstride;
     const int rows_per_round = gridDim.x * W;
     const int bpr = (n + 511) / 512;
+    const int64_t pitch = (int64_t)bpr * 512;
     const int my_rows = (n - (int)blockIdx.x * W + rows_per_round - 1) / rows_per_round;
-    const int total = my_rows * bpr;
-    auto fetch = [&](int bq, uint32_t (&lab)[8], double2 (&xv)[8]) {
-        const int rr = bq / bpr, bb = bq - rr * bpr;
-        const int r = blockIdx.x * W + rr * rows_per_round + wave;
-        const uint32_t* col = L + (int64_t)((bq < total && r < n) ? r : 0) * n;
-#pragma unroll
-        for (int u = 0; u < 8; ++u) {
-            const int c = bb * 512 + u * 64 + lane;
-            const int cc = c < n ? c : n - 1;
-            lab[u] = col[cc];
-            xv[u] = X[cc];
-        }
+    const int row0 = blockIdx.x * W + wave;
+    auto fetch = [&](const BatchCursor& c, LabelBatch<BYTES>& lab) {
+        const int r = row0 + c.rr * rows_per_round;
+        lab.load(L, n, pitch, (c.rr < my_rows && r < n) ? r : 0, c.bb, lane);
     };
-    auto process = [&](int bq, const uint32_t (&lab)[8], const double2 (&xv)[8]) {
-        if (bq >= total) return;
-        const int rr = bq / bpr, bb = bq - rr * bpr;
+    auto fetch_x = [&](const BatchCursor& c, PairBatch& xv) {
+        const double2* xb = X + c.bb * 512 + lane;
+        if ((c.bb + 1) * 512 <= n) {
+#pragma unroll
+            for (int u = 0; u < 8; ++u) xv.v[u] = xb[u * 64];
+        } else {
+#pragma unroll
+            for (int u = 0; u < 8; ++u) xv.v[u] = xb[c.bb * 512 + u * 64 + lane < n ? u * 64 : n - 1 - (c.bb * 512 + lane)];
+        }
+    };
+    auto add_entry = [&](uint32_t label, const double2& v) {
+        const uint32_t l = WIN ? window_label(label, first, (uint32_t)d) : label;
+        double2 t = mine[l];
+        t.x += v.x;
+        t.y += v.y;
+        mine[l] = t;
+    };
+    auto process = [&](const BatchCursor& cur, const LabelBatch<BYTES>& lab, const PairBatch& xv) {
+        if (cur.rr >= my_rows) return;
+        const int rr = cur.rr, bb = cur.bb;
         if (bb == 0)
             for (int i = 0; i <= d; ++i) mine[i] = make_double2(0.0, 0.0);
-#pragma unroll
-        for (int u = 0; u < 8; ++u) {
-            const int c = bb * 512 + u * 64 + lane;
-            if (c < n) {
-                const uint32_t l = WIN ? window_label(lab[u], first, (uint32_t)d) : lab[u];
-                double2 t = mine[l];
-                t.x += xv[u].x;
-                t.y += xv[u].y;
-                mine[l] = t;
-            }
+        if ((bb + 1) * 512 <= n) {
+#pragma unroll
+            for (int u = 0; u < 8; ++u) add_entry(lab.label(u), xv.v[u]);
+        } else {
+#pragma unroll
+            for (int u = 0; u < 8; ++u)
+                if (bb * 512 + u * 64 + lane < n) add_entry(lab.label(u), xv.v[u]);
         }
         if (bb == bpr - 1) {
-            const int r = blockIdx.x * W + rr * rows_per_round + wave;
+            const int r = row0 + rr * rows_per_round;
             __syncthreads();
             if (r < n)
                 for (int i = 1 + lane; i <= d; i += 64) {
@@ -932,19 +1018,9 @@
             __syncthreads();
         }
     };
-    uint32_t la[8], lb[8], lc[8];
-    double2 xa[8], xb[8], xc[8];
-    fetch(0, la, xa);
-    fetch(1, lb, xb);
-#pragma unroll 1
-    for (int bq = 0; bq < total; bq += 3) {
-        fetch(bq + 2, lc, xc);
-        process(bq, la, xa);
-        fetch(bq + 3, la, xa);
-        process(bq + 1, lb, xb);
-        fetch(bq + 4, lb, xb);
-        process(bq + 2, lc, xc);
-    }
+    BatchRing<CS2_NBUF_U32, CS2_NBUF_U32, LabelBatch<BYTES>, PairBatch> ring;
+    ring.prime(bpr, fetch, fetch_x);
+    ring.run(my_rows, bpr, fetch, fetch_x, process);
 }
 
 __global__ void __launch_bounds__(256)
@@ -1224,14 +1300,12 @@
 
 bool blockdiag_set_device_attributes() {
     bool ok = true;
-    ok &= hipSuccess == hipFuncSetAttribute(reinterpret_cast<const void*>(&class_sums2_kernel<4, false>), hipFuncAttributeMaxDynamicSharedMemorySize, 150 * 1024);
-    ok &= hipSuccess == hipFuncSetAttribute(reinterpret_cast<const void*>(&class_sums2_kernel<4, true>), hipFuncAttributeMaxDynamicSharedMemorySize, 150 * 1024);
-    ok &= hipSuccess == hipFuncSetAttribute(reinterpret_cast<const void*>(&class_sums2_kernel<2, false>), hipFuncAttributeMaxDynamicSharedMemorySize, 150 * 1024);
-    ok &= hipSuccess == hipFuncSetAttribute(reinterpret_cast<const void*>(&class_sums2_kernel<2, true>), hipFuncAttributeMaxDynamicSharedMemorySize, 150 * 1024);
-    ok &= hipSuccess == hipFuncSetAttribute(reinterpret_cast<const void*>(&class_sums2_kernel<1, false>), hipFuncAttributeMaxDynamicSharedMemorySize, 150 * 1024);
-    ok &= hipSuccess == hipFuncSetAttribute(reinterpret_cast<const void*>(&class_sums2_kernel<1, true>), hipFuncAttributeMaxDynamicSharedMemorySize, 150 * 1024);
-    ok &= hipSuccess == hipFuncSetAttribute(reinterpret_cast<const void*>(&class_sums_small_d_kernel),
-                        hipFuncAttributeMaxDynamicSharedMemorySize, 150 * 1024);
+    const void* tables[] = {
+        reinterpret_cast<const void*>(&class_sums2_kernel<4, false>), reinterpret_cast<const void*>(&class_sums2_kernel<4, true>),
+        reinterpret_cast<const void*>(&class_sums2_kernel<2, false>), reinterpret_cast<const void*>(&class_sums2_kernel<2, true>),
+        reinterpret_cast<const void*>(&class_sums2_kernel<1, false>), reinterpret_cast<const void*>(&class_sums2_kernel<1, true>),
+        reinterpret_cast<const void*>(&class_sums_small_d_kernel<false>), reinterpret_cast<const void*>(&class_sums_small_d_kernel<true>)};
+    for (const void* k : tables) ok &= hipSuccess == hipFuncSetAttribute(k, hipFuncAttributeMaxDynamicSharedMemorySize, 150 * 1024);
     ok &= hipSuccess == hipFuncSetAttribute(reinterpret_cast<const void*>(&small_qtaq_block_norms_kernel),
                         hipFuncAttributeMaxDynamicSharedMemorySize, 104 * 1024);
     ok &= hipSuccess == hipFuncSetAttribute(reinterpret_cast<const void*>(&small_cluster_qtaq_block_norms_kernel),
@@ -1249,13 +1323,19 @@
     const int tstride = (int)((d + 1) | 1);
     return ldo == n || ((size_t)n + (size_t)4 * 64 * tstride) * sizeof(double) <= 150 * 1024;
 }
-void launch_class_sums(hipStream_t s, int64_t n, int64_t d, const uint32_t* L, const double* x, double* out, int64_t ldo, uint32_t first) {
+void launch_class_sums(hipStream_t s, int64_t n, int64_t d, const uint32_t* L, const double* x, double* out, int64_t ldo, uint32_t first,
+                       const LaneBytes& lb) {
     const int tstride = (int)((d + 1) | 1);
     const size_t lds_small = ((size_t)n + (size_t)4 * 64 * tstride) * sizeof(double);
     if (lds_small <= 150 * 1024) {
         int g = (int)((n + 3) / 4);
         if (g > 256) g = 256;
-        class_sums_small_d_kernel<<<g, 256, lds_small, s>>>((int)n, (int)d, first, tstride, L, x, out, ldo);
+        if (lb.p && first == 1u && d <= 255) {
+            class_sums_small_d_kernel<true><<<g, 256, lds_small, s>>>((int)n, (int)d, first, tstride, lb.p, x, out, ldo);
+            if (lb.launches) ++*lb.launches;
+        } else {
+            class_sums_small_d_kernel<false><<<g, 256, lds_small, s>>>((int)n, (int)d, first, tstride, L, x, out, ldo);
+        }
         return;
     }
     const size_t lds = (size_t)2 * (d + 2) * 4 + (size_t)n * 2 + 16;
diff --git a/sdpsymmetryreduction.jl_amd/csrc/loop.cpp b/sdpsymmetryreduction.jl_amd/csrc/loop.cpp
--- a/sdpsymmetryreduction.jl_amd/csrc/loop.cpp
+++ b/sdpsymmetryreduction.jl_amd/csrc/loop.cpp
@@ -182,6 +182,7 @@
                 }
                 g0.sq_pass = true, g0.sq = q;
                 c->labels_on_record = rec_full;
+                c->labels8_on_record = rec_full8;
             }
         } else {
             *(volatile uint32_t*)hv = 0u;
@@ -457,6 +458,7 @@
     }
     bool initial_packed = false;
     const uint32_t* rec_full = nullptr;
+    const uint8_t* rec_full8 = nullptr;
     int square_buffers() {
         static const struct { const char *x, *c; size_t xb, cb; } B[] = {{"adm_xi8", "adm_ci32", 1, 4}, {"adm_xf32", "adm_cf32", 4, 4}, {"adm_xf64", "adm_cf64", 8, 8}};
         if (mode < SDPSR_SQUARE_I8 || mode > SDPSR_SQUARE_F64) return ctx_fail(c, SDPSR_BAD_ARGUMENT, "unknown square_mode");
@@ -558,6 +560,9 @@
     const bool record_labels = c->record_labels_allowed && c->allow_deferred_verdict && c->pinned_small && !tm.enabled && first_joint && (hint & 2) &&
                                lp.mode == SDPSR_SQUARE_I8 && !(c->opts.flags & (SDPSR_FLAG_CHECKS_IN_LOOP | SDPSR_FLAG_SQUARE_EVERY_VERDICT));
     if (guess_initial && record_labels && rec.Lfull && rec.Lfull == (const uint32_t*)ctx_buf(c, "adm_lfull_rec", (size_t)len * 4)) lp.rec_full = rec.Lfull;
+    const size_t len8 = (size_t)n * lane_bytes_pitch(n);
+    const bool record_bytes = !(c->opts.flags & SDPSR_FLAG_WIDE_BLOCKDIAG_LABELS);
+    if (lp.rec_full && record_bytes && rec.Lfull8 && rec.d0 <= 255 && rec.Lfull8 == (const uint8_t*)ctx_buf(c, "adm_lfull8_rec", len8)) lp.rec_full8 = rec.Lfull8;
     int64_t d = 0;
     tm.begin(SDPSR_T_REFINE);
     st = lp.initial_partition(dCL, dX0, hint, guess_initial ? &rec : nullptr, &d);
@@ -604,14 +609,25 @@
             if (copy && hipMemcpyAsync(copy, lp.lab.L, (size_t)len * 4, hipMemcpyDeviceToDevice, s) == hipSuccess) lfull = copy;
             else (void)hipGetLastError();
         }
+        const uint8_t* lfull8 = (guess_initial && lfull == rec.Lfull && record_bytes) ? rec.Lfull8 : nullptr;
+        if (lfull && !lfull8 && record_labels && record_bytes && c->adm_dims[0] <= 255) {
+            uint8_t* bytes = (uint8_t*)ctx_buf(c, "adm_lfull8_rec", len8);
+            if (bytes) {
+                launch_lane_order_bytes(s, n, lfull, bytes);
+                lfull8 = bytes;
+            } else {
+                c->err.clear();
+            }
+        }
         InitialRecord& ir = c->initial_record;
         ir.first = (const uint32_t*)ctx_buf(c, "ref_first", (size_t)refine_first_cap() * 4);
-        ir.Lfull = lfull;
+        ir.Lfull = lfull, ir.Lfull8 = lfull8;
         ir.n = n, ir.d0 = c->adm_dims[0], ir.Lp = lp.lab.Lp, ir.sym = lp.lab.sym;
         ir.narrow = lp.lab.narrow(), ir.Lp8 = ir.narrow ? lp.lab.Lp8 : nullptr;
         ir.valid = ir.first != nullptr;
     } else {
         c->labels_on_record = nullptr;
+        c->labels8_on_record = nullptr;
     }
     *dim_out = lp.current;
     if (iters_out) *iters_out = lp.it;
diff --git a/sdpsymmetryreduction.jl_amd/csrc/prof/prof.cpp b/sdpsymmetryreduction.jl_amd/csrc/prof/prof.cpp
--- a/sdpsymmetryreduction.jl_amd/csrc/prof/prof.cpp
+++ b/sdpsymmetryreduction.jl_amd/csrc/prof/prof.cpp
@@ -373,6 +373,15 @@
     return SDPSR_OK;
 }
 
+extern "C" int sdpsr_profile_record_bytes(sdpsr_ctx* c, int32_t restart, uint64_t* out) {
+    const int st = sdpsr_profile_recorded_labels(c, restart, out);
+    if (st) return st;
+    sdpsr_ctx* r = restart == 0 ? c : c->batch_children[restart - 1];
+    out[11] = r->check_stats.byte_class_sums;
+    out[12] = r->initial_record.valid && r->initial_record.Lfull8 ? 1 : 0;
+    return SDPSR_OK;
+}
+
 extern "C" int sdpsr_profile_square_check(sdpsr_ctx* c, int64_t n, int64_t d, int G, int T, const uint64_t* keys, int width, int write_full,
                                           const uint32_t* Lp_host, const uint32_t* first_idx_host, uint8_t* ws_inout, uint64_t* layout,
                                           uint32_t* verdicts_out, uint32_t* L_inout, int64_t guard) {
@@ -714,6 +723,44 @@
     HIP_TRY(c, hipMemcpyAsync(out_inout, out, on * 8, hipMemcpyDeviceToHost, s));
     HIP_TRY(c, hipStreamSynchronize(s));
     HIP_TRY(c, hipGetLastError());
+    return SDPSR_OK;
+}
+
+extern "C" int sdpsr_profile_class_sums_bytes(sdpsr_ctx* c, int which, int64_t n, int64_t d, uint32_t first, int plain, int use_bytes,
+                                              const uint32_t* L_host, const double* X_host, double* Y_inout, int64_t guard, uint8_t* bytes_inout,
+                                              int32_t* report) {
+    CHECK_CTX(c);
+    if (!L_host || !X_host || !Y_inout || !report || (which != 1 && which != 2) || n < 1 || n > MK_MAX_N || d < 1 || d > 4000 || first < 1 ||
+        (plain != 0 && plain != 1) || (plain && first != 1) || (use_bytes != 0 && use_bytes != 1) || guard < 0 || guard > MK_MAX_GUARD)
+        return ctx_fail(c, SDPSR_BAD_ARGUMENT, "class_sums_bytes: bad arguments");
+    const int tstride = (int)((d + 1) | 1);
+    if (which == 2 && (size_t)64 * tstride * 16 > 150 * 1024) return ctx_fail(c, SDPSR_BAD_ARGUMENT, "class_sums_bytes: no instance for this many classes");
+    const bool table1 = ((size_t)n + (size_t)4 * 64 * tstride) * 8 <= 150 * 1024;
+    if (which == 1 && !table1 && !basis_image_two_stage_fits(n, d, 1)) return ctx_fail(c, SDPSR_BAD_ARGUMENT, "class_sums_bytes: the fallback does not take this shape");
+    if ((plain || (which == 1 && first == 1 && table1)) && !mk_labels_ok(L_host, (size_t)n * n, d)) return ctx_fail(c, SDPSR_BAD_ARGUMENT, "class_sums_bytes: a label exceeds d");
+    hipStream_t s = c->stream;
+    const size_t k = (size_t)which, yn = k * n * d + (size_t)guard, bn = (size_t)n * lane_bytes_pitch(n) + (size_t)guard * 8;
+    uint32_t* Lb = (uint32_t*)ctx_buf(c, "prof_l", (size_t)n * n * 4);
+    uint8_t* B = (uint8_t*)ctx_buf(c, "prof_l8", bn);
+    double* X = (double*)ctx_buf(c, "prof_mk_a", k * n * 8);
+    double* Y = (double*)ctx_buf(c, "prof_mk_c", yn * 8);
+    if (!Lb || !B || !X || !Y) return SDPSR_OUT_OF_MEMORY;
+    HIP_TRY(c, hipMemcpyAsync(Lb, L_host, (size_t)n * n * 4, hipMemcpyHostToDevice, s));
+    HIP_TRY(c, hipMemcpyAsync(X, X_host, k * n * 8, hipMemcpyHostToDevice, s));
+    HIP_TRY(c, hipMemcpyAsync(Y, Y_inout, yn * 8, hipMemcpyHostToDevice, s));
+    if (bytes_inout) HIP_TRY(c, hipMemcpyAsync(B, bytes_inout, bn, hipMemcpyHostToDevice, s));
+    launch_lane_order_bytes(s, n, Lb, B);
+    uint64_t ran = 0;
+    const LaneBytes lb{use_bytes ? B : nullptr, &ran};
+    int W = 1;
+    if (which == 1) launch_class_sums(s, n, d, Lb, X, Y, n, first, lb);
+    else W = launch_class_sums_pair(s, n, d, first, plain != 0, Lb, X, Y);
+    HIP_TRY(c, hipMemcpyAsync(Y_inout, Y, yn * 8, hipMemcpyDeviceToHost, s));
+    if (bytes_inout) HIP_TRY(c, hipMemcpyAsync(bytes_inout, B, bn, hipMemcpyDeviceToHost, s));
+    HIP_TRY(c, hipStreamSynchronize(s));
+    HIP_TRY(c, hipGetLastError());
+    if (!W) return ctx_fail(c, SDPSR_BAD_ARGUMENT, "class_sums_bytes: no instance for this many classes");
+    report[0] = (int32_t)ran, report[1] = W;
     return SDPSR_OK;
 }
 
diff --git a/sdpsymmetryreduction.jl_amd/csrc/reduce.cpp b/sdpsymmetryreduction.jl_amd/csrc/reduce.cpp
--- a/sdpsymmetryreduction.jl_amd/csrc/reduce.cpp
+++ b/sdpsymmetryreduction.jl_amd/csrc/reduce.cpp
@@ -28,6 +28,7 @@
     c->bd_q_valid = false;
     c->bd_qrm_current = false;
     c->bd_labels_ext = nullptr;
+    c->bd_lane_bytes = nullptr;
     double pm_a[SDPSR_T_COUNT] = {}, pm_b[SDPSR_T_COUNT] = {}, pm_i[SDPSR_T_COUNT] = {};
     int labels_sym = 0;
     c->deferred_verdict = false;
@@ -74,12 +75,15 @@
     c->allow_deferred_verdict = !(c->opts.flags & SDPSR_FLAG_WAIT_FOR_EVERY_VERDICT);
     c->record_labels_allowed = in_place && !phase_ms && !(c->opts.flags & SDPSR_FLAG_LABELS_BEFORE_BLOCKDIAG);
     c->labels_on_record = nullptr;
+    c->labels8_on_record = nullptr;
     st = admissible_subspace_impl(c, n, CL, X0L, U, r, atol, L, dim_out, iters_out, phase_ms ? pm_a : nullptr, mem_in, SDPSR_MEM_DEVICE,
                                   false, &labels_sym);
     c->allow_deferred_verdict = false;
     c->record_labels_allowed = false;
     const uint32_t* Lbd = c->labels_on_record ? c->labels_on_record : L;
+    const uint8_t* Lbd8 = c->labels_on_record ? c->labels8_on_record : nullptr;
     c->labels_on_record = nullptr;
+    c->labels8_on_record = nullptr;
     const int st_loop = st;
     if (st && st != SDPSR_NOT_CONVERGED) return leave(st);
     const bool overflow = P_out && label_width_overflows(c, (uint64_t)*dim_out);
@@ -93,7 +97,7 @@
     if (!overflow && Lbd != L) ++c->check_stats.on_record;
     st = overflow ? SDPSR_OK
                   : block_diagonalize_impl(c, n, Lbd, d, epsilon, &nb, &S, &S1, phase_ms ? pm_b : nullptr, SDPSR_MEM_DEVICE, labels_sym != 0,
-                                           false, in_place);
+                                           false, in_place, true, Lbd8);
     flush_deferred_tail(c);
     if (nblocks) *nblocks = nb;
     if (sum_sq) *sum_sq = S;
@@ -109,6 +113,7 @@
             bool ok = false;
             ~Forget() {
                 c->bd_labels_ext = nullptr;
+                c->bd_lane_bytes = nullptr;
                 c->bd_trusted_symmetric = nullptr;
                 if (!ok) c->bd_valid = false;
             }
diff --git a/sdpsymmetryreduction.jl_amd/csrc/sdpsr_internal.h b/sdpsymmetryreduction.jl_amd/csrc/sdpsr_internal.h
--- a/sdpsymmetryreduction.jl_amd/csrc/sdpsr_internal.h
+++ b/sdpsymmetryreduction.jl_amd/csrc/sdpsr_internal.h
@@ -97,6 +97,7 @@
     uint64_t window_t0 = 0;
     uint32_t voided[3] = {0, 0, 0};
     uint64_t on_record = 0;
+    uint64_t byte_class_sums = 0;
 };
 constexpr uint32_t DEFERRED_NEVER_RAN = 0xDEFE44EDu;
 struct InitialRecord {
@@ -107,6 +108,7 @@
     bool narrow = false;
     const uint8_t* Lp8 = nullptr;
     const uint32_t* Lfull = nullptr;
+    const uint8_t* Lfull8 = nullptr;
 };
 constexpr int STATUS_REPEAT_REDUCTION = -0x5250;
 }
@@ -144,6 +146,7 @@
     uint32_t bd_sym_epoch = 0;
     const uint32_t* bd_sym_labels = nullptr;
     const uint32_t* bd_labels_ext = nullptr;
+    const uint8_t* bd_lane_bytes = nullptr;
     const uint32_t* bd_trusted_symmetric = nullptr;
     uint32_t epoch_counter = 0;
     const uint32_t* first_idx_labels = nullptr;
@@ -174,6 +177,7 @@
     bool initial_guess_pending = false;
     bool record_labels_allowed = false;
     const uint32_t* labels_on_record = nullptr;
+    const uint8_t* labels8_on_record = nullptr;
     uint64_t initial_guesses = 0, initial_guesses_violated = 0;
     uint64_t label_narrowings = 0;
     bool symflag_zero = false;
@@ -521,8 +525,15 @@
                               const double* Qrm, const uint32_t* ent, const int64_t* cls_ptr,
                               const int32_t* blk_col, const int32_t* blk_size, const int64_t* blk_off, double atol,
                               double* out);
+struct LaneBytes {
+    const uint8_t* p = nullptr;
+    uint64_t* launches = nullptr;
+};
+size_t lane_bytes_pitch(int64_t n);
+void launch_lane_order_bytes(hipStream_t s, int64_t n, const uint32_t* L, uint8_t* B);
 bool class_sums_supports(int64_t n, int64_t d, int64_t ldo);
-void launch_class_sums(hipStream_t s, int64_t n, int64_t d, const uint32_t* L, const double* x, double* out, int64_t ldo, uint32_t first = 1);
+void launch_class_sums(hipStream_t s, int64_t n, int64_t d, const uint32_t* L, const double* x, double* out, int64_t ldo, uint32_t first = 1,
+                       const LaneBytes& lb = {});
 int launch_class_sums_pair(hipStream_t s, int64_t n, int64_t d, uint32_t first, bool plain, const uint32_t* L, const double* X, double* Y);
 void launch_basis_image_two_stage(hipStream_t s, int64_t n, int64_t d, uint32_t first, int64_t S1, int64_t S,
                                   const uint32_t* L, const double* Qrm, double* T, const int32_t* colA,
```

Measured after the change: 2557 (median of 6 runs). 1.02x the previous value.
